# nalinbhardwaj/curdleproofs.pie

Measured on AMD Instinct MI355X. Metric: BLS12-381 G1 scalar-muls/sec at MSM size 2^20, higher is better.
Workload: dtype u32

## Files before the change

### curdleproofs_pie_amd/csrc/host_chains.h

```cpp
#pragma once

namespace cg1 {

static WinPlan make_plan(int c, bool glv = false) {
  WinPlan pl;
  const int bits = glv ? 127 : 255;
  pl.glv = glv ? 1 : 0;
  if (c > 0) { pl.cmax = c; pl.nwin = bits / c + 1; pl.n_hi = pl.nwin; }
  else {
    const int cm = -c, nw = (bits + 1 + cm - 1) / cm;
    pl.cmax = cm; pl.nwin = nw; pl.n_hi = bits + 1 - nw * (cm - 1);
    if (pl.n_hi < 0) pl.n_hi = 0;
  }
  return pl;
}

static int pick_plan_c(size_t n, int auto_plan) {
  const int c = pick_window(n);
  if (!auto_plan || c != 16) return c;
  if (n <= (1u << 14)) return -12;
  if (n <= (3u << 15)) return -13;
  if (n <= (3u << 16)) return -15;
  return 16;
}

int pick_window(size_t n) {
  if (n <= 128) return 4;
  if (n <= 8192) return 8;
  return 16;
}

static int wait_stream(Ctx* ctx) {
  if (ctx->blocking_sync) {
    HIPCHK(hipEventRecord(ctx->sync_ev, ctx->stream));
    HIPCHK(hipEventSynchronize(ctx->sync_ev));
    return CG1_OK;
  }
  HIPCHK(hipStreamSynchronize(ctx->stream));
  return CG1_OK;
}

struct PtSrc {
  enum Kind { AFFINE96 = 0, BLOBS = 1, PREPARED = 2 } kind = AFFINE96;
  const void* p = nullptr;
  const uint8_t* flags = nullptr;
  bool normalised = false;
  PtSrc() {}
  PtSrc(const void* affine96) : p(affine96) {}
};

static uint32_t blob_points_per_lane(size_t n) {
  size_t K = (n + (1u << 17) - 1) >> 17;
  return (uint32_t)(K < 1 ? 1 : (K > 16 ? 16 : K));
}

static void launch_prepare(hipStream_t st, const PtSrc& src, PreparedPoint* out, uint8_t* flags_out, uint32_t n32, uint32_t* status_words) {
  if (src.kind == PtSrc::AFFINE96) {
    hipLaunchKernelGGL(k_prepare_points, dim3((n32 + 255) / 256), dim3(256), 0, st, (const uint32_t*)src.p, out, flags_out, n32, status_words);
  } else if (src.normalised) {
    hipLaunchKernelGGL((k_prepare_blobs<false>), dim3((n32 + 127) / 128), dim3(128), 0, st, (const uint32_t*)src.p, out, flags_out, n32, 1u, status_words);
  } else {
    const uint32_t K = blob_points_per_lane(n32);
    const uint32_t lanes = (n32 + K - 1) / K;
    hipLaunchKernelGGL((k_prepare_blobs<true>), dim3((lanes + 127) / 128), dim3(128), 0, st, (const uint32_t*)src.p, out, flags_out, n32, K, status_words);
  }
}

struct ChainHooks {
  hipEvent_t before_start = nullptr, after_prepare = nullptr, before_accumulate = nullptr, after_accumulate = nullptr;
};

static int msm_enqueue(Ctx* ctx, const PtSrc& src, const void* d_scalars32, size_t n, const WinPlan& plan, int rank, int world,
                       const ChainHooks& hooks = ChainHooks()) {
  ctx->pend.active = false;
  HIPCHK(hipSetDevice(ctx->device));
  const int c = plan.cmax, nwin = plan.nwin;
  const size_t n_real = n;
  if (plan.glv) n *= 2;
  const int nlw = win_count(nwin, rank, world);
  if (nlw <= 0) return CG1_OK;
  const uint32_t NB = 1u << (c - 1);
  const uint32_t m = std::min<uint32_t>(ctx->seg_m, NB);
  const uint32_t J = NB / m;
  int nbits = 0; while ((1u << nbits) < J) ++nbits;
  const uint32_t bb = (uint32_t)c - 1u, lb2 = (bb + 1u) / 2u, hb2 = bb - lb2;
  const bool use2d = ctx->reduce_2d != 0;
  const uint32_t nitems = use2d ? 1u + hb2 + lb2 : 1u + (uint32_t)nbits;
  const size_t nb_total = (size_t)nlw * NB;
  uint32_t L0 = ctx->L0;
  while (L0 < 65536u && ((uint64_t)n * (uint64_t)nlw >> 18) > (uint64_t)L0) L0 <<= 1;
  if (ctx->chunk_rule && world == 1) {
    const uint64_t entries = (uint64_t)n * (uint64_t)nlw;
    if (entries >= (1ull << 20) && entries < (1ull << 21) && L0 < 10u) L0 = 10u;
    if (entries >= (1ull << 21) && entries < (1ull << 24) && nb_total > (size_t)ctx->rowcol_quad_max) {
      const double mload = (double)n / (double)(1u << bb);
      uint32_t want = (uint32_t)(mload + 8.0 * std::sqrt(mload) + 1.0);
      if (entries < (1ull << 22) && want > 20u) want = 20u;
      if (want > L0) L0 = want;
    }
  }
  int rc = ensure(ctx, n, nb_total, nlw, nitems, L0, src.kind != PtSrc::PREPARED);
  if (rc) return rc;
  hipStream_t st = ctx->stream;
  const uint32_t n32 = (uint32_t)n;
  const uint32_t gn = (n32 + 255) / 256;
  const int profile = ctx->profile;
  auto h0 = std::chrono::steady_clock::now();
  const bool resident = src.kind == PtSrc::PREPARED;
  const PreparedPoint* pts = resident ? static_cast<const PreparedPoint*>(src.p) : ctx->d_pts;
  const uint8_t* flags = resident ? src.flags : ctx->d_flags;
  const size_t nout_words = (size_t)nlw * nitems;
  uint32_t* bad_flag = reinterpret_cast<uint32_t*>(ctx->d_out + nout_words);
  if (hooks.before_start) HIPCHK(hipStreamWaitEvent(st, hooks.before_start, 0));
  if (profile >= 2) HIPCHK(hipEventRecord(ctx->ev[0], st));
  const uint32_t n_real32 = (uint32_t)n_real;
  if (resident) HIPCHK(hipMemsetAsync(bad_flag, 0, 16, st));
  else {
    launch_prepare(st, src, ctx->d_pts, ctx->d_flags, n_real32, bad_flag);
    if (plan.glv) hipLaunchKernelGGL(k_phi_records, dim3((n_real32 + 255) / 256), dim3(256), 0, st, ctx->d_pts, ctx->d_flags, n_real32);
  }
  if (hooks.after_prepare) HIPCHK(hipEventRecord(hooks.after_prepare, st));
  if (profile >= 2) HIPCHK(hipEventRecord(ctx->ev[1], st));
  const uint32_t nblk = (uint32_t)((nb_total + SCAN_ITEMS - 1) / SCAN_ITEMS);
  if (ctx->use_partition_sort && n <= PART_MAX_N) {
    const uint32_t want_sub = ctx->sort_sub_bits ? (uint32_t)ctx->sort_sub_bits : (n <= ((size_t)1 << 16) ? 7u : 8u);
    uint32_t sub_bits = bb < want_sub ? bb : want_sub;
    while (bb - sub_bits > 7u) ++sub_bits;
    const uint32_t nbins = 1u << (bb - sub_bits);
    const uint32_t nslices = (n32 + PART_TILE - 1) / PART_TILE;
    const uint32_t nbc = (uint32_t)nlw * nbins * nslices;
    hipLaunchKernelGGL(k_digits, dim3((n_real32 + 255) / 256), dim3(256), 0, st, (const uint32_t*)d_scalars32, flags, ctx->d_digits, n_real32, plan, rank, world, bad_flag);
    hipLaunchKernelGGL(k_part_count, dim3(nslices, nlw), dim3(256), 0, st, ctx->d_digits, ctx->d_blockcnt, n32, nslices, nbins, sub_bits);
    const uint32_t ublk = (nbc + SCAN_ITEMS - 1) / SCAN_ITEMS;
    if (ctx->scan_one && nbc <= USCAN1_MAX) {
      hipLaunchKernelGGL(k_uscan_one, dim3(1), dim3(1024), 0, st, ctx->d_blockcnt, nbc);
    } else {
      hipLaunchKernelGGL(k_uscan1, dim3(ublk), dim3(256), 0, st, ctx->d_blockcnt, ctx->d_ublocktot, nbc);
      hipLaunchKernelGGL(k_uscan2, dim3(1), dim3(256), 0, st, ctx->d_ublocktot, ublk, ctx->d_blockcnt, nbc);
      hipLaunchKernelGGL(k_uscan3, dim3(ublk), dim3(256), 0, st, ctx->d_ublocktot, ctx->d_blockcnt, nbc);
    }
    if (profile >= 2) HIPCHK(hipEventRecord(ctx->ev[2], st));
    hipLaunchKernelGGL(k_part_scatter, dim3(nslices, nlw), dim3(256), 0, st, ctx->d_digits, ctx->d_blockcnt, ctx->d_part, n32, nslices, nbins, sub_bits, ctx->stage_sort);
    const uint32_t nbt = (uint32_t)nlw * nbins;
    const int big_bins = ctx->big_bins && n32 > 2u * BIN_STAGE;
    hipLaunchKernelGGL(k_slice_plan, dim3(1), dim3(256), 0, st, ctx->d_blockcnt, nbt, nslices, ctx->d_slice_base, ctx->d_bigflag, big_bins);
    hipLaunchKernelGGL(k_bin_sort, dim3(nbt), dim3(256), 0, st, ctx->d_part, ctx->d_blockcnt, ctx->d_hist, ctx->d_sorted, nbt, nslices, sub_bits, ctx->stage_sort, ctx->d_bigflag);
    if (big_bins) {
      const uint32_t max_slices = (uint32_t)(((size_t)n * (size_t)nlw) / SLICE + nbt + 1);
      hipLaunchKernelGGL(k_slice_count, dim3(max_slices), dim3(256), 0, st, ctx->d_part, ctx->d_blockcnt, nbt, nslices, ctx->d_slice_base, ctx->d_slicehist);
      hipLaunchKernelGGL(k_slice_prefix, dim3(nbt), dim3(256), 0, st, ctx->d_blockcnt, nslices, sub_bits, ctx->d_slice_base, ctx->d_bigflag, ctx->d_slicehist, ctx->d_subbase, ctx->d_hist);
      hipLaunchKernelGGL(k_slice_scatter, dim3(max_slices), dim3(256), 0, st, ctx->d_part, ctx->d_blockcnt, nbt, nslices, ctx->d_slice_base, ctx->d_slicehist, ctx->d_subbase, ctx->d_sorted);
    }
    if (profile >= 2) HIPCHK(hipEventRecord(ctx->ev[3], st));
    if (ctx->scan_one && nb_total <= SCAN1_MAX) {
      hipLaunchKernelGGL(k_scan_one, dim3(1), dim3(1024), 0, st, ctx->d_hist, ctx->d_off, ctx->d_choff, (uint32_t)nb_total, L0);
    } else {
      hipLaunchKernelGGL(k_scan1, dim3(nblk), dim3(256), 0, st, ctx->d_hist, ctx->d_off, ctx->d_choff, ctx->d_blocktot, (uint32_t)nb_total, L0);
      hipLaunchKernelGGL(k_scan2, dim3(1), dim3(256), 0, st, ctx->d_blocktot, nblk, ctx->d_off, ctx->d_choff, (uint32_t)nb_total);
      hipLaunchKernelGGL(k_scan3, dim3(nblk), dim3(256), 0, st, ctx->d_blocktot, ctx->d_off, ctx->d_choff, (uint32_t)nb_total);
    }
  } else {
    HIPCHK(hipMemsetAsync(ctx->d_hist, 0, nb_total * 4, st));
    hipLaunchKernelGGL(k_hist, dim3(gn), dim3(256), 0, st, (const uint32_t*)d_scalars32, flags, ctx->d_hist, n32, plan, rank, world, bad_flag);
    if (profile >= 2) HIPCHK(hipEventRecord(ctx->ev[2], st));
    hipLaunchKernelGGL(k_scan1, dim3(nblk), dim3(256), 0, st, ctx->d_hist, ctx->d_off, ctx->d_choff, ctx->d_blocktot, (uint32_t)nb_total, L0);
    hipLaunchKernelGGL(k_scan2, dim3(1), dim3(256), 0, st, ctx->d_blocktot, nblk, ctx->d_off, ctx->d_choff, (uint32_t)nb_total);
    hipLaunchKernelGGL(k_scan3, dim3(nblk), dim3(256), 0, st, ctx->d_blocktot, ctx->d_off, ctx->d_choff, (uint32_t)nb_total);
    if (profile >= 2) HIPCHK(hipEventRecord(ctx->ev[3], st));
    hipLaunchKernelGGL(k_scatter, dim3(gn), dim3(256), 0, st, (const uint32_t*)d_scalars32, flags, ctx->d_hist, ctx->d_off, ctx->d_sorted, n32, plan, rank, world);
  }
  HIPCHK(hipMemsetAsync(ctx->d_zblock, 0, zblock_clear_bytes(ctx), st));
  hipLaunchKernelGGL(k_chunk_desc, dim3((uint32_t)std::min<size_t>(CHUNK_DESC_BLOCKS, (nb_total + 255) / 256)), dim3(256), 0, st, ctx->d_off, ctx->d_choff, ctx->d_desc, ctx->d_lenhist, ctx->d_heavy, (uint32_t)ctx->cap_heavy, (uint32_t)nb_total, L0, ctx->d_any_multi);
  const size_t max_chunks = nb_total + (n * (size_t)nlw) / L0 + 1;
  const uint32_t gchunks = (uint32_t)((max_chunks + 255) / 256);
  hipLaunchKernelGGL(k_len_scan, dim3(1), dim3(256), 0, st, ctx->d_lenhist, ctx->d_lenhist + LEN_BINS, ctx->d_off + nb_total, ctx->d_choff + nb_total, bad_flag);
  hipLaunchKernelGGL(k_order, dim3((gchunks + ORDER_PER - 1) / ORDER_PER), dim3(256), 0, st, ctx->d_desc, ctx->d_choff + nb_total, ctx->d_lenhist + LEN_BINS, ctx->d_order);
  if (hooks.before_accumulate) HIPCHK(hipStreamWaitEvent(st, hooks.before_accumulate, 0));
  if (profile >= 1) HIPCHK(hipEventRecord(ctx->ev[4], st));
  hipLaunchKernelGGL(k_accumulate, dim3(gchunks), dim3(256), 0, st, ctx->d_desc, ctx->d_choff + nb_total, ctx->d_order, ctx->d_sorted, pts, ctx->d_sums);
  if (profile >= 1) HIPCHK(hipEventRecord(ctx->ev[5], st));
  if (hooks.after_accumulate) HIPCHK(hipEventRecord(hooks.after_accumulate, st));
  hipLaunchKernelGGL(k_heavy_combine, dim3(512), dim3(256), 0, st, ctx->d_heavy, (uint32_t)ctx->cap_heavy, ctx->d_choff, ctx->d_sums, ctx->d_combined);
  const bool small_quad = ctx->quad && ctx->rowcol_quad && nb_total <= (size_t)ctx->rowcol_quad_max;
  const bool rows_fold = small_quad && use2d && ctx->rowcol_row && ctx->tree_row && nb_total <= 8192;
  if (rows_fold) {}
  else if (small_quad && ctx->fold_quad)
    hipLaunchKernelGGL(k_bucket_fold_quad, dim3((uint32_t)((nb_total * 4 + 255) / 256)), dim3(256), 0, st, ctx->d_choff, ctx->d_sums, ctx->d_combined, (uint32_t)nb_total, ctx->d_any_multi);
  else if (ctx->fold_pass)
    hipLaunchKernelGGL(k_bucket_fold, dim3((uint32_t)((nb_total + 255) / 256)), dim3(256), 0, st, ctx->d_choff, ctx->d_sums, ctx->d_combined, (uint32_t)nb_total, ctx->d_any_multi);
  bool tree_exports = false;
  if (use2d) {
    const uint32_t R = 1u << hb2, Cn = 1u << lb2;
    const uint32_t lpr = Cn < 32u ? Cn : 32u, lpc = R < 16u ? R : 16u;
    const uint32_t nrow_blocks = ((uint32_t)nlw * R + (256u / lpr) - 1u) / (256u / lpr);
    const uint32_t ncol_blocks = ((uint32_t)nlw * Cn + (256u / lpc) - 1u) / (256u / lpc);
    PointSum* rowsum = ctx->d_segrun;
    PointSum* colsum = ctx->d_segtot;
    if (small_quad) {
      uint32_t lgq = (R == Cn) ? 2u : 3u;
      if (ctx->rowcol_lgq >= 2 && ctx->rowcol_lgq <= 4) lgq = (uint32_t)ctx->rowcol_lgq;
      const uint32_t rc_waves = ((uint32_t)nlw * (R + Cn) + (16u >> lgq) - 1u) / (16u >> lgq);
      if (ctx->rowcol_row && ctx->tree_row)
        hipLaunchKernelGGL(k_rowcol_quad_row, dim3(((uint32_t)nlw * (R + Cn) + 3u) / 4u), dim3(256), 0, st, ctx->d_choff, ctx->d_sums, ctx->d_combined,
                           rowsum, colsum, (uint32_t)nlw, hb2, lb2);
      else
      hipLaunchKernelGGL(k_rowcol_quad, dim3((rc_waves + 3u) / 4u), dim3(256), 0, st, ctx->d_choff, ctx->d_sums,
                         rowsum, colsum, (uint32_t)nlw, hb2, lb2, lgq);
    }
    else
      hipLaunchKernelGGL(k_rowcol, dim3(nrow_blocks + ncol_blocks), dim3(256), 0, st, ctx->d_choff, ctx->d_sums, ctx->d_combined,
                         rowsum, colsum, (uint32_t)nlw, hb2, lb2, nrow_blocks, ctx->quad);
    if (profile >= 2) HIPCHK(hipEventRecord(ctx->ev[6], st));
    const uint32_t tree_threads = std::min<uint32_t>(512u, std::max<uint32_t>(64u, 4u << std::max(hb2, lb2)) >> (ctx->tree_shift >= 0 ? ctx->tree_shift : (ctx->tree_half ? 1 : 0)));
    if (ctx->tree_row) {
      uint32_t W = (1u << std::max(hb2, lb2)) >> 3;
      W = W < 1u ? 1u : (W > 16u ? 16u : W);
      tree_exports = ctx->zero_copy != 0;
      if (tree_exports) ++ctx->seq;
      hipLaunchKernelGGL(k_small_tree_row, dim3(nitems, nlw), dim3(64u * W), 0, st, rowsum, colsum, ctx->d_out, hb2, lb2,
                         tree_exports ? ctx->h_out_dev : (PointWords*)nullptr, bad_flag, ctx->h_flag_dev, ctx->seq);
    }
    else if (ctx->quad) hipLaunchKernelGGL(k_small_tree_quad, dim3(nitems, nlw), dim3(std::max<uint32_t>(64u, tree_threads)), 0, st, rowsum, colsum, ctx->d_out, hb2, lb2);
    else hipLaunchKernelGGL(k_small_tree, dim3(nitems, nlw), dim3(256), 0, st, rowsum, colsum, ctx->d_out, hb2, lb2);
  } else {
    const uint32_t nseg_total = (uint32_t)(nb_total / m);
    hipLaunchKernelGGL(k_seg_reduce, dim3((nseg_total + 255) / 256), dim3(256), 0, st, ctx->d_choff, ctx->d_sums, ctx->d_combined, ctx->d_segrun, ctx->d_segtot, nseg_total, m);
    if (profile >= 2) HIPCHK(hipEventRecord(ctx->ev[6], st));
    uint32_t S = (J + BT_ELEMS - 1) / BT_ELEMS; if (S < 1) S = 1; if (S > 64) S = 64;
    hipLaunchKernelGGL(k_bit_tree, dim3(nitems, nlw, S), dim3(256), 0, st, ctx->d_segrun, ctx->d_segtot, ctx->d_partial, J);
    hipLaunchKernelGGL(k_bit_tree_final, dim3((uint32_t)(nitems * nlw)), dim3(64), 0, st, ctx->d_partial, ctx->d_out, S);
  }
  const bool zc = ctx->zero_copy != 0;
  if (zc && tree_exports) {
  } else if (zc) {
    ++ctx->seq;
    const uint32_t nvec = (uint32_t)((((size_t)nlw * nitems + 1) * sizeof(PointWords)) / 16);
    hipLaunchKernelGGL(k_export_host, dim3(1), dim3(1024), 0, st, reinterpret_cast<const uint4*>(ctx->d_out), reinterpret_cast<uint4*>(ctx->h_out_dev), nvec,
                       ctx->h_flag_dev, ctx->seq);
  } else {
    HIPCHK(hipMemcpyAsync(ctx->h_out, ctx->d_out, ((size_t)nlw * nitems + 1) * sizeof(PointWords), hipMemcpyDeviceToHost, st));
  }
  if (profile >= 2) HIPCHK(hipEventRecord(ctx->ev[7], st));
  auto h1 = std::chrono::steady_clock::now();
  Ctx::Pending& pd = ctx->pend;
  pd.zero_copy = zc; pd.seq = ctx->seq; pd.hout = ctx->h_out;
  pd.active = true; pd.c = c; pd.plan = plan; pd.rank = rank; pd.world = world; pd.nlw = nlw; pd.nbits = nbits; pd.m = m; pd.lb2 = lb2; pd.hb2 = hb2;
  pd.nitems = nitems; pd.use2d = use2d; pd.profile = profile; pd.nout_words = nout_words; pd.h0 = h0; pd.h1 = h1;
  pd.arm_helpers = ctx->arm_helpers && ctx->host_split && ctx->horner_threads > 1 && n <= ((size_t)1 << 18);
  return CG1_OK;
}

static int msm_finish(Ctx* ctx, cg1h::jac& result) {
  result = cg1h::jac_identity();
  if (!ctx->pend.active) return CG1_OK;
  const Ctx::Pending pd = ctx->pend;
  ctx->pend.active = false;
  const int c = pd.c, rank = pd.rank, world = pd.world, nlw = pd.nlw, nbits = pd.nbits;
  (void)c;
  const uint32_t m = pd.m, lb2 = pd.lb2, hb2 = pd.hb2, nitems = pd.nitems;
  const bool use2d = pd.use2d;
  const size_t nout_words = pd.nout_words;
  const auto h0 = pd.h0, h1 = pd.h1;
  HIPCHK(hipSetDevice(ctx->device));
  struct StandDown { Ctx* c; bool on; ~StandDown() { if (on) for (int j = 0; j < 3; ++j) c->helper[j].disarm(); } } stand_down{ctx, false};
  if (pd.zero_copy && !ctx->blocking_sync && pd.profile < 2) {
    if (pd.arm_helpers) for (int j = 0; j < 3 && j + 1 < ctx->horner_threads; ++j) ctx->helper[j].arm();
    stand_down.on = pd.arm_helpers;
    volatile uint32_t* flag = ctx->h_flag;
    for (uint32_t spins = 0; *flag != pd.seq; ++spins) {
      if ((spins & 0x3fffu) == 0x3fffu) {
        hipError_t q = hipStreamQuery(ctx->stream);
        if (q == hipSuccess) { if (*flag != pd.seq) { snprintf(ctx->err, sizeof ctx->err, "the stream drained without the export flag"); return CG1_ERR_HIP; } break; }
        if (q != hipErrorNotReady) { snprintf(ctx->err, sizeof ctx->err, "stream failed: %s", hipGetErrorString(q)); return CG1_ERR_HIP; }
      }
      __builtin_ia32_pause();
    }
    std::atomic_thread_fence(std::memory_order_acquire);
  } else {
    int wrc = wait_stream(ctx); if (wrc) return wrc;
  }
  HIPCHK(hipGetLastError());
  {
    const uint32_t* st_words = reinterpret_cast<const uint32_t*>(pd.hout + nout_words);
    ctx->last_entries = st_words[1]; ctx->last_chunks = st_words[2];
    if (st_words[0]) {
      snprintf(ctx->err, sizeof ctx->err, "a scalar is >= 2^255: scalar32 must be a canonical Fr element (< r)");
      return CG1_ERR_ENCODING;
    }
  }
  auto h2 = std::chrono::steady_clock::now();
  { int erc = read_phase_events(ctx, pd.profile); if (erc) return erc; }
  ctx->last_c = c;

  auto t0 = std::chrono::steady_clock::now();
  ctx->host_ms[0] = std::chrono::duration<float, std::milli>(h1 - h0).count();
  ctx->host_ms[1] = std::chrono::duration<float, std::milli>(h2 - h1).count();
  ctx->host_ms[2] = std::chrono::duration<float, std::milli>(t0 - h2).count();
  int lm = 0; while ((1u << lm) < m) ++lm;
  const WinPlan& plan = pd.plan;
  constexpr int EMAX = 2 * 256 + 64;
  std::vector<std::pair<int, const PointWords*>> items;
  items.reserve((size_t)nlw * nitems);
  int e_top = 0;
  for (int lw = 0; lw < nlw; ++lw) {
    const int w = win_global(lw, rank, world), base = plan.off(w);
    const PointWords* row = pd.hout + (size_t)lw * nitems;
    auto put = [&](int e, const PointWords* p) { if (!p->inf && e >= 0 && e < EMAX) { items.emplace_back(e, p); if (e > e_top) e_top = e; } };
    put(base, &row[0]);
    if (use2d) {
      for (uint32_t k = 0; k < hb2; ++k) put(base + (int)lb2 + (int)k, &row[1 + k]);
      for (uint32_t k = 0; k < lb2; ++k) put(base + (int)k, &row[1 + hb2 + k]);
    } else {
      for (int b2 = 0; b2 < nbits; ++b2) put(base + lm + b2, &row[1 + b2]);
    }
  }
  uint16_t first[EMAX + 1];
  memset(first, 0, sizeof first);
  for (const auto& it : items) ++first[it.first + 1];
  for (int e = 0; e < EMAX; ++e) first[e + 1] = (uint16_t)(first[e + 1] + first[e]);
  std::vector<const PointWords*> byexp(items.size());
  {
    uint16_t cur[EMAX];
    memcpy(cur, first, sizeof cur);
    for (const auto& it : items) byexp[cur[it.first]++] = it.second;
  }
  auto horner = [&](int lo, int hi) {
    cg1h::jac a = cg1h::jac_identity();
    for (int e = hi; e >= lo; --e) {
      a = cg1h::jac_dbl(a);
      for (uint16_t k = first[e]; k < first[e + 1]; ++k) a = cg1h::jac_add(a, jac_from_words(*byexp[k]));
    }
    return a;
  };
  cg1h::jac acc;
  const int nth = (!ctx->host_split || e_top < 96) ? 1 : (ctx->horner_threads >= 4 && e_top >= 112 ? 4 : 2);
  if (nth > 1) {
    cg1h::jac part[4];
    int lo[5];
    {
      constexpr long DBL = 7, ADD = 16;
      auto fill = [&](long C, int* cut) {
        int e = 0;
        for (int j = 0; j < nth; ++j) {
          cut[j] = e;
          long adds = 0;
          while (e <= e_top && DBL * (e + 1) + ADD * (adds + (first[e + 1] - first[e])) <= C) { adds += first[e + 1] - first[e]; ++e; }
        }
        cut[nth] = e_top + 1;
        return e > e_top;
      };
      long lo_c = DBL * (e_top + 1), hi_c = DBL * (e_top + 1) + ADD * (long)items.size();
      int cut[5];
      while (lo_c < hi_c) {
        const long mid = (lo_c + hi_c) / 2;
        if (fill(mid, cut)) hi_c = mid; else lo_c = mid + 1;
      }
      fill(hi_c, cut);
      for (int j = 0; j <= nth; ++j) lo[j] = cut[j];
    }
    auto run_part = [&](int j) {
      cg1h::jac a = horner(lo[j], lo[j + 1] - 1);
      for (int k = 0; k < lo[j]; ++k) a = cg1h::jac_dbl(a);
      part[j] = a;
    };
    for (int j = 0; j + 1 < nth; ++j) ctx->helper[j].run([&, j]() { run_part(j); });
    if (pd.arm_helpers) for (int j = nth - 1 < 0 ? 0 : nth - 1; j < 3; ++j) ctx->helper[j].disarm();
    run_part(nth - 1);
    acc = part[nth - 1];
    for (int j = 0; j + 1 < nth; ++j) { ctx->helper[j].wait(); acc = cg1h::jac_add(acc, part[j]); }
  } else {
    if (pd.arm_helpers) for (int j = 0; j < 3; ++j) ctx->helper[j].disarm();
    acc = horner(0, e_top);
  }
  result = acc;
  ctx->host_tail_ms = std::chrono::duration<float, std::milli>(std::chrono::steady_clock::now() - t0).count();
  ctx->host_ms[3] = ctx->host_tail_ms;
  return CG1_OK;
}

static int pick_small_c(size_t n) {
  if (n <= 24) return 4;
  if (n <= 96) return 6;
  if (n <= 6 * SM_SLICE) return 7;
  return 8;
}

static int msm_enqueue_small(Ctx* ctx, const PtSrc& src, const void* d_scalars32, size_t n, int c, uint32_t M = 1, const uint32_t* d_offs = nullptr, size_t max_n = 0,
                             bool glv = false) {
  ctx->pend.active = false;
  HIPCHK(hipSetDevice(ctx->device));
  const WinPlan plan = make_plan(c, glv);
  const uint32_t nwin = (uint32_t)plan.nwin, bb = (uint32_t)c - 1u, lb2 = (bb + 1u) / 2u, hb2 = bb - lb2, nitems = 1u + hb2 + lb2;
  if (M == 1) max_n = n;
  const uint32_t S = (uint32_t)(((glv ? 2 * max_n : max_n) + SM_SLICE - 1) / SM_SLICE);
  auto h0 = std::chrono::steady_clock::now();
  if (!ctx->h_small_out) {
    HIPCHK(hipHostMalloc((void**)&ctx->h_small_out, ((size_t)SM_MAX_MSMS * 64 * 9 + 1) * sizeof(PointWords), hipHostMallocMapped | hipHostMallocCoherent));
    HIPCHK(hipHostGetDevicePointer((void**)&ctx->h_small_out_dev, ctx->h_small_out, 0));
    HIPCHK(hipMalloc(&ctx->d_small_ctr, (SM_MAX_MSMS * 64 + 8) * 4));
    HIPCHK(hipMemsetAsync(ctx->d_small_ctr, 0, (SM_MAX_MSMS * 64 + 8) * 4, ctx->stream));
  }
  const size_t need_partial = (size_t)M * nwin * S * nitems;
  if (S > 1 && need_partial > ctx->cap_small_partial) {
    if (ctx->d_small_partial) (void)hipFree(ctx->d_small_partial);
    ctx->d_small_partial = nullptr; ctx->cap_small_partial = 0;
    HIPCHK(hipMalloc(&ctx->d_small_partial, need_partial * sizeof(PointSum)));
    ctx->cap_small_partial = need_partial;
  }
  hipStream_t st = ctx->stream;
  SmallArgs a;
  a.src = src.p; a.flags = src.flags; a.scalars = static_cast<const uint32_t*>(d_scalars32); a.offs = d_offs;
  a.n = (uint32_t)n; a.M = M; a.S = S; a.c = (uint32_t)c; a.nwin = nwin; a.hb = hb2; a.lb = lb2; a.nitems = nitems;
  a.partial = ctx->d_small_partial; a.counters = ctx->d_small_ctr;
  a.out_host = ctx->h_small_out_dev; a.flag_host = ctx->h_flag_dev; a.seq = ++ctx->seq;
  a.row_tail = ctx->small_row_tail ? 1u : 0u;
  a.glv = glv ? 1u : 0u;
  int kind = (int)src.kind;
  if (src.kind == PtSrc::BLOBS && !src.normalised) {
    if (n > ctx->cap_small_pts) {
      if (ctx->d_small_pts) (void)hipFree(ctx->d_small_pts);
      if (ctx->d_small_flags) (void)hipFree(ctx->d_small_flags);
      ctx->d_small_pts = nullptr; ctx->d_small_flags = nullptr; ctx->cap_small_pts = 0;
      const size_t cap = n < SM_MAX_N ? SM_MAX_N : n;
      HIPCHK(hipMalloc(&ctx->d_small_pts, cap * sizeof(PreparedPoint)));
      HIPCHK(hipMalloc(&ctx->d_small_flags, cap + 16));
      ctx->cap_small_pts = cap;
    }
    launch_prepare(st, src, ctx->d_small_pts, ctx->d_small_flags, (uint32_t)n, nullptr);
    a.src = ctx->d_small_pts; a.flags = ctx->d_small_flags;
    kind = (int)PtSrc::PREPARED;
  }
  const dim3 grid(nwin, S, M), block(512);
  if (kind == (int)PtSrc::AFFINE96) hipLaunchKernelGGL((k_msm_small<0>), grid, block, 0, st, a);
  else if (kind == (int)PtSrc::BLOBS) hipLaunchKernelGGL((k_msm_small<1>), grid, block, 0, st, a);
  else hipLaunchKernelGGL((k_msm_small<2>), grid, block, 0, st, a);
  auto h1 = std::chrono::steady_clock::now();
  Ctx::Pending& pd = ctx->pend;
  pd.zero_copy = true; pd.seq = ctx->seq; pd.hout = ctx->h_small_out;
  pd.active = true; pd.c = c; pd.plan = plan; pd.rank = 0; pd.world = 1; pd.nlw = (int)nwin; pd.nbits = 0; pd.m = 1; pd.lb2 = lb2; pd.hb2 = hb2;
  pd.nitems = nitems; pd.use2d = true; pd.profile = 0; pd.nout_words = (size_t)M * nwin * nitems; pd.h0 = h0; pd.h1 = h1;
  pd.arm_helpers = ctx->arm_helpers && ctx->host_split && ctx->horner_threads > 1 && M == 1;
  return CG1_OK;
}

static cg1h::jac horner_2d_items(const PointWords* rows, const WinPlan& plan, uint32_t nitems, uint32_t hb2, uint32_t lb2) {
  constexpr int EMAX = 2 * 256 + 64;
  std::vector<std::pair<int, const PointWords*>> items;
  items.reserve((size_t)plan.nwin * nitems);
  int e_top = 0;
  for (int w = 0; w < plan.nwin; ++w) {
    const int base = plan.off(w);
    const PointWords* row = rows + (size_t)w * nitems;
    auto put = [&](int e, const PointWords* p) { if (!p->inf) { items.emplace_back(e, p); if (e > e_top) e_top = e; } };
    put(base, &row[0]);
    for (uint32_t k = 0; k < hb2; ++k) put(base + (int)lb2 + (int)k, &row[1 + k]);
    for (uint32_t k = 0; k < lb2; ++k) put(base + (int)k, &row[1 + hb2 + k]);
  }
  uint16_t first[EMAX + 1];
  memset(first, 0, sizeof first);
  for (const auto& it : items) ++first[it.first + 1];
  for (int e = 0; e < EMAX; ++e) first[e + 1] = (uint16_t)(first[e + 1] + first[e]);
  std::vector<const PointWords*> byexp(items.size());
  {
    uint16_t cur[EMAX];
    memcpy(cur, first, sizeof cur);
    for (const auto& it : items) byexp[cur[it.first]++] = it.second;
  }
  cg1h::jac a = cg1h::jac_identity();
  for (int e = e_top; e >= 0; --e) {
    a = cg1h::jac_dbl(a);
    for (uint16_t k = first[e]; k < first[e + 1]; ++k) a = cg1h::jac_add(a, jac_from_words(*byexp[k]));
  }
  return a;
}

static int msm_small_batched_finish(Ctx* ctx, uint32_t M, std::vector<cg1h::jac>& results) {
  const Ctx::Pending pd = ctx->pend;
  ctx->pend.active = false;
  HIPCHK(hipSetDevice(ctx->device));
  if (!ctx->blocking_sync) {
    volatile uint32_t* flag = ctx->h_flag;
    for (uint32_t spins = 0; *flag != pd.seq; ++spins) {
      if ((spins & 0x3fffu) == 0x3fffu) {
        hipError_t q = hipStreamQuery(ctx->stream);
        if (q == hipSuccess) { if (*flag != pd.seq) { snprintf(ctx->err, sizeof ctx->err, "the stream drained without the export flag"); return CG1_ERR_HIP; } break; }
        if (q != hipErrorNotReady) { snprintf(ctx->err, sizeof ctx->err, "stream failed: %s", hipGetErrorString(q)); return CG1_ERR_HIP; }
      }
      __builtin_ia32_pause();
    }
    std::atomic_thread_fence(std::memory_order_acquire);
  } else {
    int wrc = wait_stream(ctx); if (wrc) return wrc;
  }
  HIPCHK(hipGetLastError());
  const uint32_t* st_words = reinterpret_cast<const uint32_t*>(pd.hout + pd.nout_words);
  ctx->last_entries = st_words[1]; ctx->last_chunks = 0;
  if (st_words[0]) {
    snprintf(ctx->err, sizeof ctx->err, "a scalar is >= 2^255: scalar32 must be a canonical Fr element (< r)");
    return CG1_ERR_ENCODING;
  }
  auto t0 = std::chrono::steady_clock::now();
  const size_t per = (size_t)pd.plan.nwin * pd.nitems;
  auto one = [&](size_t j) { results[j] = horner_2d_items(pd.hout + j * per, pd.plan, pd.nitems, pd.hb2, pd.lb2); };
  if (M <= 4) {
    const size_t nth = std::min<size_t>(4, M);
    for (size_t t = 1; t < nth; ++t) ctx->helper[t - 1].run([&, t]() { for (size_t j = t; j < M; j += nth) one(j); });
    for (size_t j = 0; j < M; j += nth) one(j);
    for (size_t t = 1; t < nth; ++t) ctx->helper[t - 1].wait();
  } else {
    std::atomic<size_t> next{0};
    std::function<void()> work = [&]() { for (;;) { const size_t j = next.fetch_add(1); if (j >= M) return; one(j); } };
    Pool& pool = Pool::get();
    pool.run(work, std::min<size_t>(M, pool.size() + 1));
  }
  auto t1 = std::chrono::steady_clock::now();
  ctx->host_ms[0] = std::chrono::duration<float, std::milli>(pd.h1 - pd.h0).count();
  ctx->host_ms[1] = std::chrono::duration<float, std::milli>(t0 - pd.h1).count();
  ctx->host_ms[2] = 0;
  ctx->host_ms[3] = ctx->host_tail_ms = std::chrono::duration<float, std::milli>(t1 - t0).count();
  for (int i = 0; i < CG1_NPHASE; ++i) ctx->phase_ms[i] = 0.f;
  ctx->last_c = pd.c;
  ctx->last_acc_launches = 0;
  return CG1_OK;
}

static Ctx* child_of(Ctx* ctx);
static int msm_begin_split(Ctx* ctx, const PtSrc& src, const void* d_scalars32, size_t n, const WinPlan& plan, int rank, int world);

int msm_begin(Ctx* ctx, const PtSrc& src, const void* d_scalars32, size_t n, int c, int rank, int world) {
  ctx->pend.active = false;
  ctx->pend_c = 0;
  if (n == 0) return CG1_OK;
  if (n >= (1ull << 31)) { snprintf(ctx->err, sizeof ctx->err, "n too large"); return CG1_ERR_ARG; }
  if (world < 1 || world > 255 || rank < 0 || rank >= world) { snprintf(ctx->err, sizeof ctx->err, "bad window shard %d/%d", rank, world); return CG1_ERR_ARG; }
  for (int pass = (ctx->glv && 2 * n <= SM_MAX_N) ? 1 : 0; pass >= 0; --pass) {
    const bool sglv = pass == 1;
    const size_t nn = sglv ? 2 * n : n;
    const int bits = sglv ? 127 : 255;
    if (ctx->small_msm && nn <= SM_MAX_N && world == 1 && (c == 0 || (c >= 4 && c <= 9 && c != 5)) &&
        (size_t)(bits / (c ? c : pick_small_c(nn)) + 1) * ((nn + SM_SLICE - 1) / SM_SLICE) <= SM_ONE_ROUND) {
      if (c == 0) c = pick_small_c(nn);
      ctx->pend_c = c;
      return msm_enqueue_small(ctx, src, d_scalars32, n, c, 1, nullptr, 0, sglv);
    }
  }
  const bool glv = src.kind != PtSrc::PREPARED && ctx->use_partition_sort && 2 * n <= PART_MAX_N &&
                   (ctx->glv == 2 || (ctx->glv == 1 && n <= (size_t)ctx->glv_max_n));
  if (c == 0) c = pick_plan_c(glv ? 2 * n : n, ctx->auto_plan);
  const int cabs = c < 0 ? -c : c;
  if (cabs < 4 || cabs > 16) { snprintf(ctx->err, sizeof ctx->err, "window width %d out of range [4,16]", c); return CG1_ERR_ARG; }
  const WinPlan plan = make_plan(c, glv);
  ctx->pend_c = c;
  ctx->pend_split = false;
  if (ctx->split && n >= ctx->split_min_n && win_count(plan.nwin, rank, world) >= 2) return msm_begin_split(ctx, src, d_scalars32, n, plan, rank, world);
  return msm_enqueue(ctx, src, d_scalars32, n, plan, rank, world);
}
int msm_end(Ctx* ctx, cg1h::jac& result) {
  const bool was_small = ctx->pend.active && ctx->pend.hout == ctx->h_small_out;
  int rc = msm_finish(ctx, result);
  ctx->last_acc_launches = ctx->pend_split ? 2 : (was_small ? 0 : 1);
  if (ctx->pend_split) {
    ctx->pend_split = false;
    Ctx* ch = child_of(ctx);
    const float acc_hi = ctx->phase_ms[4], wait_hi = ctx->host_ms[1], tail_hi = ctx->host_ms[3], enq = ctx->host_ms[0];
    const uint32_t e_hi = ctx->last_entries, c_hi = ctx->last_chunks;
    cg1h::jac lo;
    int rc2 = msm_finish(ch, lo);
    if (rc == CG1_OK) rc = rc2;
    if (rc2 != CG1_OK) snprintf(ctx->err, sizeof ctx->err, "%s", ch->err);
    if (rc == CG1_OK) result = cg1h::jac_add(result, lo);
    for (int i = 0; i < CG1_NPHASE; ++i) ctx->phase_ms[i] += ch->phase_ms[i];
    ctx->phase_ms[4] = acc_hi + ch->phase_ms[4];
    ctx->last_entries = e_hi + ch->last_entries; ctx->last_chunks = c_hi + ch->last_chunks;
    ctx->host_ms[0] = enq + ch->host_ms[0]; ctx->host_ms[1] = wait_hi + ch->host_ms[1]; ctx->host_ms[3] = tail_hi + ch->host_ms[3];
    ctx->host_tail_ms = ch->host_ms[3];
  }
  if (ctx->pend_c) ctx->last_c = ctx->pend_c;
  return rc;
}
int msm_device(Ctx* ctx, const PtSrc& src, const void* d_scalars32, size_t n, int c, int rank, int world, cg1h::jac& result) {
  result = cg1h::jac_identity();
  int rc = msm_begin(ctx, src, d_scalars32, n, c, rank, world);
  if (rc) return rc;
  return msm_end(ctx, result);
}


int pick_window_batched(size_t n_avg, bool glv) {
  const int bits = glv ? 127 : 255;
  if (glv) n_avg *= 2;
  int best = 4; double best_cost = 1e300;
  for (int c = 4; c <= 9; ++c) {
    if (bits % c == 0) continue;
    int nwin = bits / c + 1;
    double NB = (double)(1u << (c - 1));
    double cost = (double)nwin * ((double)n_avg + 1.4 * (2.0 * NB + 3.0 * NB / 8.0)) + 1.4 * (double)bits;
    if (cost < best_cost) { best_cost = cost; best = c; }
  }
  return best;
}
int pick_window_batched(size_t n_avg) { return pick_window_batched(n_avg, false); }

static int ensure_child(Ctx* ctx);

struct BatchedChain {
  size_t M = 0; int c = 0; uint32_t nwin = 0; bool host_horner = false;
  std::chrono::steady_clock::time_point h0, h1;
};
static int batched_chain_enqueue(Ctx* ctx, const void* d_points96, const void* d_scalars32, const uint32_t* h_offsets, size_t M, int c, bool glv,
                                 hipEvent_t wait_before_accumulate, hipEvent_t record_after_accumulate, BatchedChain& bc) {
  const size_t N = h_offsets[M], N_real = N;
  HIPCHK(hipSetDevice(ctx->device));
  const WinPlan bplan = make_plan(c, glv);
  const uint32_t nwin = (uint32_t)bplan.nwin, NB = 1u << (c - 1);
  const size_t G = M * nwin, nb_total = G * NB;
  const size_t Nv = glv ? 2 * N : N;
  if (nb_total >= (1ull << 31) || Nv * nwin >= (1ull << 31)) { snprintf(ctx->err, sizeof ctx->err, "batch too large"); return CG1_ERR_ARG; }
  const uint32_t m = 8 < NB ? 8 : NB;
  uint32_t log2m = 0; while ((1u << log2m) < m) ++log2m;
  const uint32_t J = NB / m;
  uint32_t L0 = ctx->L0;
  while (L0 < 65536u && ((uint64_t)Nv * (uint64_t)nwin >> 18) > (uint64_t)L0) L0 <<= 1;
  int rc = ensure(ctx, Nv, nb_total, nwin, 1, L0);
  if (rc) return rc;
  if ((M + 1) > ctx->cap_boffs) {
    if (ctx->d_boffs) (void)hipFree(ctx->d_boffs);
    HIPCHK(hipMalloc(&ctx->d_boffs, (M + 1) * 4));
    ctx->cap_boffs = M + 1;
  }
  if (G > ctx->cap_gsum) {
    if (ctx->d_gsum) (void)hipFree(ctx->d_gsum);
    HIPCHK(hipMalloc(&ctx->d_gsum, G * sizeof(PointSum)));
    ctx->cap_gsum = G;
  }
  if (M > ctx->cap_bout) {
    if (ctx->d_bout) (void)hipFree(ctx->d_bout);
    if (ctx->h_bout) (void)hipHostFree(ctx->h_bout);
    HIPCHK(hipMalloc(&ctx->d_bout, (M + 1) * sizeof(PointWords)));
    HIPCHK(hipHostMalloc(&ctx->h_bout, (M + 1) * sizeof(PointWords)));
    ctx->cap_bout = M;
  }
  if (Nv * nwin > ctx->cap_digits) {
    if (ctx->d_digits) (void)hipFree(ctx->d_digits);
    HIPCHK(hipMalloc(&ctx->d_digits, Nv * nwin * 2 + 16));
    ctx->cap_digits = Nv * nwin;
  }
  hipStream_t st = ctx->stream;
  const uint32_t N32 = (uint32_t)N_real, gn = (N32 + 255) / 256, Nv32 = (uint32_t)Nv, split = glv ? N32 : 0u;
  auto h0 = std::chrono::steady_clock::now();
  HIPCHK(hipMemcpyAsync(ctx->d_boffs, h_offsets, (M + 1) * 4, hipMemcpyHostToDevice, st));
  if (ctx->profile >= 2) HIPCHK(hipEventRecord(ctx->ev[0], st));
  uint32_t* bad_flag = reinterpret_cast<uint32_t*>(ctx->d_bout + M);
  hipLaunchKernelGGL(k_prepare_points, dim3(gn), dim3(256), 0, st, (const uint32_t*)d_points96, ctx->d_pts, ctx->d_flags, N32, bad_flag);
  if (glv) hipLaunchKernelGGL(k_phi_records, dim3(gn), dim3(256), 0, st, ctx->d_pts, ctx->d_flags, N32);
  if (ctx->profile >= 2) HIPCHK(hipEventRecord(ctx->ev[1], st));
  hipLaunchKernelGGL(k_digits, dim3(gn), dim3(256), 0, st, (const uint32_t*)d_scalars32, ctx->d_flags, ctx->d_digits, N32, bplan, 0, 1, bad_flag);
  hipLaunchKernelGGL(k_group_count, dim3((uint32_t)M, nwin), dim3(256), 0, st, ctx->d_digits, ctx->d_boffs, ctx->d_hist, Nv32, NB, nwin, split);
  if (ctx->profile >= 2) HIPCHK(hipEventRecord(ctx->ev[2], st));
  const uint32_t nblk = (uint32_t)((nb_total + SCAN_ITEMS - 1) / SCAN_ITEMS);
  hipLaunchKernelGGL(k_scan1, dim3(nblk), dim3(256), 0, st, ctx->d_hist, ctx->d_off, ctx->d_choff, ctx->d_blocktot, (uint32_t)nb_total, L0);
  hipLaunchKernelGGL(k_scan2, dim3(1), dim3(256), 0, st, ctx->d_blocktot, nblk, ctx->d_off, ctx->d_choff, (uint32_t)nb_total);
  hipLaunchKernelGGL(k_scan3, dim3(nblk), dim3(256), 0, st, ctx->d_blocktot, ctx->d_off, ctx->d_choff, (uint32_t)nb_total);
  hipLaunchKernelGGL(k_group_scatter, dim3((uint32_t)M, nwin), dim3(256), 0, st, ctx->d_digits, ctx->d_boffs, ctx->d_off, ctx->d_sorted, Nv32, NB, nwin, split);
  if (ctx->profile >= 2) HIPCHK(hipEventRecord(ctx->ev[3], st));
  HIPCHK(hipMemsetAsync(ctx->d_zblock, 0, zblock_clear_bytes(ctx), st));
  hipLaunchKernelGGL(k_chunk_desc, dim3((uint32_t)std::min<size_t>(CHUNK_DESC_BLOCKS, (nb_total + 255) / 256)), dim3(256), 0, st, ctx->d_off, ctx->d_choff, ctx->d_desc, ctx->d_lenhist, ctx->d_heavy, (uint32_t)ctx->cap_heavy, (uint32_t)nb_total, L0, ctx->d_any_multi);
  const size_t max_chunks = nb_total + (Nv * (size_t)nwin) / L0 + 1;
  const uint32_t gchunks = (uint32_t)((max_chunks + 255) / 256);
  hipLaunchKernelGGL(k_len_scan, dim3(1), dim3(256), 0, st, ctx->d_lenhist, ctx->d_lenhist + LEN_BINS, ctx->d_off + nb_total, ctx->d_choff + nb_total, bad_flag);
  hipLaunchKernelGGL(k_order, dim3((gchunks + ORDER_PER - 1) / ORDER_PER), dim3(256), 0, st, ctx->d_desc, ctx->d_choff + nb_total, ctx->d_lenhist + LEN_BINS, ctx->d_order);
  if (wait_before_accumulate) HIPCHK(hipStreamWaitEvent(st, wait_before_accumulate, 0));
  if (ctx->profile >= 1) HIPCHK(hipEventRecord(ctx->ev[4], st));
  hipLaunchKernelGGL(k_accumulate, dim3(gchunks), dim3(256), 0, st, ctx->d_desc, ctx->d_choff + nb_total, ctx->d_order, ctx->d_sorted, ctx->d_pts, ctx->d_sums);
  if (ctx->profile >= 1) HIPCHK(hipEventRecord(ctx->ev[5], st));
  if (record_after_accumulate) HIPCHK(hipEventRecord(record_after_accumulate, st));
  const uint32_t nseg_total = (uint32_t)(nb_total / m);
  hipLaunchKernelGGL(k_heavy_combine, dim3(512), dim3(256), 0, st, ctx->d_heavy, (uint32_t)ctx->cap_heavy, ctx->d_choff, ctx->d_sums, ctx->d_combined);
  hipLaunchKernelGGL(k_seg_reduce, dim3((nseg_total + 255) / 256), dim3(256), 0, st, ctx->d_choff, ctx->d_sums, ctx->d_combined, ctx->d_segrun, ctx->d_segtot, nseg_total, m);
  hipLaunchKernelGGL(k_group_reduce, dim3((uint32_t)((G + 255) / 256)), dim3(256), 0, st, ctx->d_segrun, ctx->d_segtot, ctx->d_gsum, (uint32_t)G, J, log2m);
  if (ctx->profile >= 2) HIPCHK(hipEventRecord(ctx->ev[6], st));
  const bool host_horner = M <= (size_t)ctx->batched_host_horner_max;
  if (host_horner) {
    if (G > ctx->cap_gout) {
      if (ctx->d_gout) (void)hipFree(ctx->d_gout);
      if (ctx->h_gout) (void)hipHostFree(ctx->h_gout);
      ctx->d_gout = nullptr; ctx->h_gout = nullptr; ctx->cap_gout = 0;
      HIPCHK(hipMalloc(&ctx->d_gout, G * sizeof(PointWords)));
      HIPCHK(hipHostMalloc(&ctx->h_gout, G * sizeof(PointWords)));
      ctx->cap_gout = G;
    }
    hipLaunchKernelGGL(k_export_sums, dim3((uint32_t)((G + 63) / 64)), dim3(64), 0, st, ctx->d_gsum, ctx->d_gout, (uint32_t)G);
    HIPCHK(hipMemcpyAsync(ctx->h_gout, ctx->d_gout, G * sizeof(PointWords), hipMemcpyDeviceToHost, st));
    HIPCHK(hipMemcpyAsync(ctx->h_bout + M, ctx->d_bout + M, sizeof(PointWords), hipMemcpyDeviceToHost, st));
  } else {
    if (ctx->horner_row && M <= 2048) hipLaunchKernelGGL(k_msm_horner_row, dim3((uint32_t)M), dim3(64), 0, st, ctx->d_gsum, ctx->d_bout, (uint32_t)M, nwin, (uint32_t)c);
    else if (ctx->quad) hipLaunchKernelGGL(k_msm_horner_quad, dim3((uint32_t)((M * 4 + 63) / 64)), dim3(64), 0, st, ctx->d_gsum, ctx->d_bout, (uint32_t)M, nwin, (uint32_t)c);
    else hipLaunchKernelGGL(k_msm_horner, dim3((uint32_t)((M + 63) / 64)), dim3(64), 0, st, ctx->d_gsum, ctx->d_bout, (uint32_t)M, nwin, (uint32_t)c);
    HIPCHK(hipMemcpyAsync(ctx->h_bout, ctx->d_bout, (M + 1) * sizeof(PointWords), hipMemcpyDeviceToHost, st));
  }
  if (ctx->profile >= 2) HIPCHK(hipEventRecord(ctx->ev[7], st));
  bc.M = M; bc.c = c; bc.nwin = nwin; bc.host_horner = host_horner; bc.h0 = h0; bc.h1 = std::chrono::steady_clock::now();
  return CG1_OK;
}

static int batched_chain_finish(Ctx* ctx, const BatchedChain& bc, cg1h::jac* results) {
  const size_t M = bc.M; const int c = bc.c; const uint32_t nwin = bc.nwin; const bool host_horner = bc.host_horner;
  const auto h0 = bc.h0, h1 = bc.h1;
  HIPCHK(hipSetDevice(ctx->device));
  { int wrc = wait_stream(ctx); if (wrc) return wrc; }
  HIPCHK(hipGetLastError());
  {
    const uint32_t* st_words = reinterpret_cast<const uint32_t*>(ctx->h_bout + M);
    ctx->last_entries = st_words[1]; ctx->last_chunks = st_words[2];
    if (st_words[0]) {
      snprintf(ctx->err, sizeof ctx->err, "a scalar is >= 2^255: scalar32 must be a canonical Fr element (< r)");
      return CG1_ERR_ENCODING;
    }
  }
  auto h2 = std::chrono::steady_clock::now();
  { int erc = read_phase_events(ctx, ctx->profile); if (erc) return erc; }
  ctx->last_c = c;
  if (host_horner) {
    auto one = [&](size_t j) {
      cg1h::jac a = cg1h::jac_identity();
      for (int w = (int)nwin - 1; w >= 0; --w) {
        for (int k = 0; k < c; ++k) a = cg1h::jac_dbl(a);
        a = cg1h::jac_add(a, jac_from_words(ctx->h_gout[j * nwin + (size_t)w]));
      }
      results[j] = a;
    };
    const size_t nth = std::min<size_t>(4, M);
    for (size_t t = 1; t < nth; ++t) ctx->helper[t - 1].run([&, t]() { for (size_t j = t; j < M; j += nth) one(j); });
    for (size_t j = 0; j < M; j += nth) one(j);
    for (size_t t = 1; t < nth; ++t) ctx->helper[t - 1].wait();
  } else {
    for (size_t j = 0; j < M; ++j) results[j] = jac_from_words(ctx->h_bout[j]);
  }
  auto h3 = std::chrono::steady_clock::now();
  ctx->host_ms[0] = std::chrono::duration<float, std::milli>(h1 - h0).count();
  ctx->host_ms[1] = std::chrono::duration<float, std::milli>(h2 - h1).count();
  ctx->host_ms[2] = 0;
  ctx->host_ms[3] = ctx->host_tail_ms = std::chrono::duration<float, std::milli>(h3 - h2).count();
  return CG1_OK;
}

static int msm_batched_small_end(Ctx* ctx, size_t M, std::vector<cg1h::jac>& results) {
  if (M == 1) { cg1h::jac r; int rc = msm_finish(ctx, r); ctx->last_acc_launches = 0; if (rc == CG1_OK) results[0] = r; return rc; }
  return msm_small_batched_finish(ctx, (uint32_t)M, results);
}
int msm_batched_device(Ctx* ctx, const void* d_points96, const void* d_scalars32, const uint32_t* h_offsets, size_t M,
                       int c, std::vector<cg1h::jac>& results, bool* async_small = nullptr, const uint32_t* d_offsets_ready = nullptr) {
  if (async_small) *async_small = false;
  results.assign(M, cg1h::jac_identity());
  if (M == 0) return CG1_OK;
  const size_t N = h_offsets[M];
  for (size_t j = 0; j < M; ++j) if (h_offsets[j] > h_offsets[j + 1]) { snprintf(ctx->err, sizeof ctx->err, "offsets not monotone"); return CG1_ERR_ARG; }
  if (h_offsets[0] != 0) { snprintf(ctx->err, sizeof ctx->err, "offsets[0] must be 0"); return CG1_ERR_ARG; }
  if (N == 0) return CG1_OK;
  if (N >= (1ull << 31) || M > 65535) { snprintf(ctx->err, sizeof ctx->err, "batch too large"); return CG1_ERR_ARG; }
  {
    size_t max_n = 0;
    for (size_t j = 0; j < M; ++j) max_n = std::max<size_t>(max_n, h_offsets[j + 1] - h_offsets[j]);
    const bool sglv = ctx->glv && 2 * max_n <= SM_MAX_N;
    const size_t max_nn = sglv ? 2 * max_n : max_n;
    const int cs = c > 0 ? c : pick_small_c(max_nn);
    const size_t groups = (size_t)M * (size_t)((sglv ? 127 : 255) / cs + 1) * ((max_nn + SM_SLICE - 1) / SM_SLICE);
    if (ctx->small_msm && M <= SM_MAX_MSMS && max_nn <= SM_MAX_N && groups <= SM_MAX_GROUPS && cs >= 4 && cs <= 9 && cs != 5) {
      HIPCHK(hipSetDevice(ctx->device));
      const uint32_t* d_offs = d_offsets_ready;
      if (!d_offs) {
        if ((M + 1) > ctx->cap_boffs) {
          if (ctx->d_boffs) (void)hipFree(ctx->d_boffs);
          ctx->d_boffs = nullptr; ctx->cap_boffs = 0;
          HIPCHK(hipMalloc(&ctx->d_boffs, (M + 1) * 4));
          ctx->cap_boffs = M + 1;
        }
        HIPCHK(hipMemcpyAsync(ctx->d_boffs, h_offsets, (M + 1) * 4, hipMemcpyHostToDevice, ctx->stream));
        d_offs = ctx->d_boffs;
      }
      int rc = msm_enqueue_small(ctx, PtSrc(d_points96), d_scalars32, N, cs, (uint32_t)M, d_offs, max_n, sglv);
      if (rc) return rc;
      if (async_small) { *async_small = true; return CG1_OK; }
      return msm_batched_small_end(ctx, M, results);
    }
  }
  const bool glv = ctx->glv != 0 && 2 * N < (1ull << 31);
  if (c <= 0) c = pick_window_batched((N + M - 1) / M, glv);
  if (c < 4 || c > 9) { snprintf(ctx->err, sizeof ctx->err, "batched window width %d out of range [4,9]", c); return CG1_ERR_ARG; }
  HIPCHK(hipSetDevice(ctx->device));
  if (!ctx->batched_split || M < (size_t)ctx->batched_split_min_m || h_offsets[M / 2] == 0 || h_offsets[M / 2] == N) {
    BatchedChain bc;
    int rc = batched_chain_enqueue(ctx, d_points96, d_scalars32, h_offsets, M, c, glv, nullptr, nullptr, bc);
    if (rc) return rc;
    return batched_chain_finish(ctx, bc, results.data());
  }
  { int crc = ensure_child(ctx); if (crc) return crc; }
  Ctx* ch = child_of(ctx);
  ch->profile = ctx->profile; ch->L0 = ctx->L0; ch->quad = ctx->quad; ch->horner_row = ctx->horner_row; ch->blocking_sync = ctx->blocking_sync;
  ch->batched_host_horner_max = ctx->batched_host_horner_max; ch->use_partition_sort = ctx->use_partition_sort;
  const size_t Mlo = M / 2, Mhi = M - Mlo;
  std::vector<uint32_t> offs_hi(Mhi + 1);
  for (size_t j = 0; j <= Mhi; ++j) offs_hi[j] = h_offsets[Mlo + j] - h_offsets[Mlo];
  BatchedChain lo, hi;
  int rc = batched_chain_enqueue(ctx, d_points96, d_scalars32, h_offsets, Mlo, c, glv, nullptr, ctx->ev_acc, lo);
  if (rc) return rc;
  rc = batched_chain_enqueue(ch, static_cast<const uint8_t*>(d_points96) + 96ull * h_offsets[Mlo], static_cast<const uint8_t*>(d_scalars32) + 32ull * h_offsets[Mlo],
                             offs_hi.data(), Mhi, c, glv, ctx->ev_acc, nullptr, hi);
  if (rc) { snprintf(ctx->err, sizeof ctx->err, "%s", ch->err); (void)batched_chain_finish(ctx, lo, results.data()); return rc; }
  rc = batched_chain_finish(ctx, lo, results.data());
  const float acc_lo = ctx->phase_ms[4], enq_lo = ctx->host_ms[0], wait_lo = ctx->host_ms[1];
  const uint32_t e_lo = ctx->last_entries, c_lo = ctx->last_chunks;
  int rc2 = batched_chain_finish(ch, hi, results.data() + Mlo);
  if (rc2 != CG1_OK) snprintf(ctx->err, sizeof ctx->err, "%s", ch->err);
  if (rc == CG1_OK) rc = rc2;
  ctx->phase_ms[4] = acc_lo + ch->phase_ms[4];
  ctx->last_entries = e_lo + ch->last_entries; ctx->last_chunks = c_lo + ch->last_chunks;
  ctx->host_ms[0] = enq_lo + ch->host_ms[0]; ctx->host_ms[1] = wait_lo + ch->host_ms[1];
  return rc;
}

}
```

### curdleproofs_pie_amd/csrc/host_context.h

```cpp
#pragma once

namespace cg1 {

#define HIPCHK(x) do { hipError_t e_ = (x); if (e_ != hipSuccess) { \
  snprintf(ctx->err, sizeof ctx->err, "%s failed: %s (%s:%d)", #x, hipGetErrorString(e_), __FILE__, __LINE__); return CG1_ERR_HIP; } } while (0)

struct Helper {
  std::thread th;
  std::mutex mu;
  std::condition_variable cv;
  std::function<void()> job;
  bool has = false, done = true, quit = false, armed = false;
  std::atomic<bool> posted{false};
  std::atomic<bool> stand_down{false};
  void start_locked() { if (!th.joinable()) th = std::thread([this]() { loop(); }); }
  void run(std::function<void()> f) {
    std::unique_lock<std::mutex> lk(mu);
    start_locked();
    job = std::move(f); has = true; done = false;
    posted.store(true, std::memory_order_release);
    cv.notify_all();
  }
  void arm() {
    std::unique_lock<std::mutex> lk(mu);
    start_locked();
    if (!has && done) { stand_down.store(false, std::memory_order_relaxed); armed = true; cv.notify_all(); }
  }
  void disarm() { stand_down.store(true, std::memory_order_release); }
  void wait() {
    std::unique_lock<std::mutex> lk(mu);
    cv.wait(lk, [this]() { return done; });
  }
  void loop() {
    std::unique_lock<std::mutex> lk(mu);
    for (;;) {
      cv.wait(lk, [this]() { return has || quit || armed; });
      if (quit) return;
      if (!has) {
        armed = false;
        lk.unlock();
        const auto until = std::chrono::steady_clock::now() + std::chrono::milliseconds(2);
        for (uint32_t k = 0; !posted.load(std::memory_order_acquire); ++k) {
          if (stand_down.load(std::memory_order_acquire)) break;
          if ((k & 0xffu) == 0xffu && std::chrono::steady_clock::now() > until) break;
          __builtin_ia32_pause();
        }
        lk.lock();
        if (!has) continue;
      }
      armed = false;
      std::function<void()> f = std::move(job);
      has = false;
      posted.store(false, std::memory_order_relaxed);
      lk.unlock();
      f();
      lk.lock();
      done = true;
      cv.notify_all();
    }
  }
  ~Helper() {
    { std::unique_lock<std::mutex> lk(mu); quit = true; cv.notify_all(); }
    if (th.joinable()) th.join();
  }
};

struct Ctx {
  int device = 0;
  Helper helper[3];
  hipStream_t stream = nullptr;
  std::atomic<hipStream_t> copy_stream{nullptr};
  std::once_flag copy_once;
  hipEvent_t copy_ev = nullptr;
  std::vector<uint32_t> cu_mask;
  hipStream_t side_stream = nullptr;
  hipEvent_t side_ev = nullptr;
  hipEvent_t sync_ev = nullptr;
  int blocking_sync = 0;
  char err[256] = {0};
  size_t cap_n = 0, cap_nb = 0, cap_chunks = 0, cap_entries = 0, cap_out = 0;
  PreparedPoint* d_pts = nullptr;
  uint8_t* d_flags = nullptr;
  uint32_t *d_hist = nullptr, *d_off = nullptr, *d_choff = nullptr, *d_sorted = nullptr;
  uint2 *d_blocktot = nullptr, *d_desc = nullptr;
  uint32_t *d_order = nullptr, *d_lenhist = nullptr;
  uint32_t* d_zblock = nullptr; size_t cap_zblock = 0;
  uint32_t* d_any_multi = nullptr;
  PointSum* d_partial = nullptr; size_t cap_partial = 0;
  uint16_t* d_digits = nullptr; uint32_t* d_part = nullptr; uint32_t* d_blockcnt = nullptr; uint32_t* d_ublocktot = nullptr;
  size_t cap_digits = 0, cap_part = 0, cap_blockcnt = 0;
  uint32_t *d_slice_base = nullptr, *d_slicehist = nullptr, *d_subbase = nullptr; uint8_t* d_bigflag = nullptr;
  size_t cap_bigflag = 0, cap_slices = 0;
  int big_bins = 1;
  int use_partition_sort = 1;
  int stage_sort = 1;
  int host_split = 1;
  int rowcol_quad = 1;
  int rowcol_lgq = 0;
  int rowcol_quad_max = 1 << 18;
  int tree_shift = 2;
  int tree_half = 1;
  int merlin_sync = 1;
  uint32_t merlin_clk[2] = {0, 0};
  int fe_timed = 0;
  int fe_rows = 1;
  int fe_prio = 0;
  int decompress_waves = 3;
  void* d_opening = nullptr; size_t cap_opening = 0;
  void* d_prover = nullptr; size_t cap_prover = 0;
  PreparedPoint* d_gen_tab = nullptr;
  int fixed_slice = 0;
  int fixed_waves = 0;
  int ipa_inv = 0;
  int merlin_last_kernel = 0;
  int merlin_rows = 1;
  void* d_merlin_rows = nullptr; size_t merlin_rows_cap = 0;
  int merlin_lanes = 64;
  uint32_t merlin_passes = 0;
  int sort_sub_bits = 0;
  int batch_mul_host_max = -1;
  int last_batch_mul_on_host = 0;
  int batch_mul_quad_max = 8192;
  int scan_one = 1;
  int fold_pass = 1;
  int auto_plan = 1;
  struct Pending {
    bool active = false;
    int c = 0, rank = 0, world = 1, nlw = 0, nbits = 0;
    WinPlan plan;
    uint32_t m = 1, lb2 = 0, hb2 = 0, nitems = 0;
    bool use2d = true;
    int profile = 0;
    bool zero_copy = false; uint32_t seq = 0;
    bool arm_helpers = false;
    size_t nout_words = 0;
    const PointWords* hout = nullptr;
    std::chrono::steady_clock::time_point h0, h1;
  } pend;
  int split = 0;
  size_t split_min_n = (size_t)1 << 17;
  cg1_ctx* child = nullptr;
  hipEvent_t ev_prep = nullptr, ev_acc = nullptr;
  bool pend_split = false;
  int last_acc_launches = 0;
  int small_row_tail = 1;
  int small_msm = 1;
  PointSum* d_small_partial = nullptr; size_t cap_small_partial = 0;
  uint32_t* d_small_ctr = nullptr;
  PreparedPoint* d_small_pts = nullptr; uint8_t* d_small_flags = nullptr; size_t cap_small_pts = 0;
  PointWords* h_small_out = nullptr; PointWords* h_small_out_dev = nullptr;
  int quad = 1;
  int reduce_2d = 1;
  uint32_t* d_heavy = nullptr; size_t cap_heavy = 0;
  uint8_t* d_combined = nullptr; size_t cap_combined = 0;
  uint32_t* d_boffs = nullptr; size_t cap_boffs = 0;
  PointSum* d_gsum = nullptr; size_t cap_gsum = 0;
  PointWords* d_bout = nullptr; PointWords* h_bout = nullptr; size_t cap_bout = 0;
  PointWords* d_gout = nullptr; PointWords* h_gout = nullptr; size_t cap_gout = 0;
  int glv = 0;
  int glv_max_n = 1 << 14;
  int lincomb_zero_copy = 1;
  int fold_quad = 1;
  int rowcol_row = 1;
  int tree_row = 1;
  int horner_row = 1;
  int batch_mul_row = 1;
  int batched_split = 0;
  int batched_split_min_m = 256;
  int batched_host_horner_max = 24;
  PointSum *d_sums = nullptr, *d_segrun = nullptr, *d_segtot = nullptr;
  PointWords* d_out = nullptr;
  PointWords* h_out = nullptr;
  PointWords* h_out_dev = nullptr;
  uint32_t* h_flag = nullptr;
  uint32_t* h_flag_dev = nullptr;
  uint32_t seq = 0;
  int zero_copy = 1;
  int arm_helpers = 1;
  int horner_threads = 4;
  void* d_stage_pts = nullptr; void* d_stage_sc = nullptr; size_t cap_stage_pts = 0, cap_stage_sc = 0;
  uint8_t* h_lin = nullptr; uint8_t* h_lin_dev = nullptr; size_t cap_h_lin = 0;
  hipEvent_t ev[CG1_NPHASE + 1];
  float phase_ms[CG1_NPHASE] = {0};
  float host_tail_ms = 0;
  float host_ms[4] = {0, 0, 0, 0};
  int profile = 1;
  uint32_t last_chunks = 0, last_entries = 0;
  hipEvent_t tm_ev[2] = {nullptr, nullptr};
  int last_c = 0, pend_c = 0;
  int chunk_rule = 1;
  uint32_t L0 = 8;
  uint32_t seg_m = 4;
};

static void free_bufs(Ctx* c) {
  auto F = [](auto*& p) { if (p) { (void)hipFree(p); p = nullptr; } };
  F(c->d_pts); F(c->d_flags); F(c->d_hist); F(c->d_off); F(c->d_choff); F(c->d_sorted); F(c->d_blocktot); F(c->d_desc);
  F(c->d_sums); F(c->d_segrun); F(c->d_segtot); F(c->d_out); F(c->d_order); F(c->d_zblock); F(c->d_partial);
  c->d_lenhist = c->d_heavy = c->d_any_multi = nullptr; c->d_combined = nullptr; c->cap_zblock = 0; c->cap_heavy = 0; c->cap_combined = 0;
  c->cap_partial = 0;
  F(c->d_digits); F(c->d_part); F(c->d_blockcnt); F(c->d_ublocktot); F(c->d_boffs); F(c->d_gsum); F(c->d_bout);
  F(c->d_slice_base); F(c->d_slicehist); F(c->d_subbase); F(c->d_bigflag); c->cap_bigflag = 0; c->cap_slices = 0;
  if (c->h_bout) { (void)hipHostFree(c->h_bout); c->h_bout = nullptr; }
  if (c->h_lin) { (void)hipHostFree(c->h_lin); c->h_lin = nullptr; c->h_lin_dev = nullptr; c->cap_h_lin = 0; }
  if (c->d_gout) { (void)hipFree(c->d_gout); c->d_gout = nullptr; }
  if (c->h_gout) { (void)hipHostFree(c->h_gout); c->h_gout = nullptr; }
  c->cap_gout = 0;
  c->cap_boffs = c->cap_gsum = c->cap_bout = 0;
  c->cap_digits = c->cap_part = c->cap_blockcnt = 0;
  if (c->h_out) { (void)hipHostFree(c->h_out); c->h_out = nullptr; }
  c->cap_n = c->cap_nb = c->cap_chunks = c->cap_entries = c->cap_out = 0;
}

static int ensure(Ctx* ctx, size_t n, size_t nb_total, size_t nlw, size_t nitems, uint32_t L, bool need_points = true) {
  size_t entries = n * nlw;
  size_t chunks = nb_total + entries / L + 1;
  if (need_points && n > ctx->cap_n) {
    if (ctx->d_pts) (void)hipFree(ctx->d_pts);
    if (ctx->d_flags) (void)hipFree(ctx->d_flags);
    HIPCHK(hipMalloc(&ctx->d_pts, n * sizeof(PreparedPoint)));
    HIPCHK(hipMalloc(&ctx->d_flags, n + 16));
    ctx->cap_n = n;
  }
  if (nb_total > ctx->cap_nb) {
    auto F = [](auto*& p) { if (p) { (void)hipFree(p); p = nullptr; } };
    F(ctx->d_hist); F(ctx->d_off); F(ctx->d_choff); F(ctx->d_blocktot); F(ctx->d_segrun); F(ctx->d_segtot);
    HIPCHK(hipMalloc(&ctx->d_hist, nb_total * 4));
    HIPCHK(hipMalloc(&ctx->d_off, (nb_total + 1) * 4));
    HIPCHK(hipMalloc(&ctx->d_choff, (nb_total + 1) * 4));
    HIPCHK(hipMalloc(&ctx->d_blocktot, (nb_total / SCAN_ITEMS + 2) * sizeof(uint2)));
    HIPCHK(hipMalloc(&ctx->d_segrun, nb_total * sizeof(PointSum)));
    HIPCHK(hipMalloc(&ctx->d_segtot, nb_total * sizeof(PointSum)));
    ctx->cap_nb = nb_total;
  }
  if (entries > ctx->cap_entries) {
    if (ctx->d_sorted) (void)hipFree(ctx->d_sorted);
    HIPCHK(hipMalloc(&ctx->d_sorted, (entries + 1) * 4));
    ctx->cap_entries = entries;
  }
  if (chunks > ctx->cap_chunks) {
    if (ctx->d_desc) (void)hipFree(ctx->d_desc);
    if (ctx->d_sums) (void)hipFree(ctx->d_sums);
    if (ctx->d_order) (void)hipFree(ctx->d_order);
    HIPCHK(hipMalloc(&ctx->d_order, chunks * 4));
    HIPCHK(hipMalloc(&ctx->d_desc, chunks * sizeof(uint2)));
    HIPCHK(hipMalloc(&ctx->d_sums, chunks * sizeof(PointSum)));
    ctx->cap_chunks = chunks;
  }
  {
    const size_t hcap = entries / ((size_t)L * (HEAVY_MIN_CHUNKS - 1)) + 2;
    const size_t z0 = 2 * LEN_BINS + 1, h0 = z0 + (nb_total + 3) / 4, words = h0 + 1 + hcap + 64;
    if (words > ctx->cap_zblock) {
      if (ctx->d_zblock) (void)hipFree(ctx->d_zblock);
      ctx->d_zblock = nullptr; ctx->cap_zblock = 0;
      HIPCHK(hipMalloc(&ctx->d_zblock, words * 4));
      ctx->cap_zblock = words;
    }
    ctx->d_lenhist = ctx->d_zblock;
    ctx->d_any_multi = ctx->d_zblock + 2 * LEN_BINS;
    ctx->d_combined = reinterpret_cast<uint8_t*>(ctx->d_zblock + z0);
    ctx->d_heavy = ctx->d_zblock + h0;
    ctx->cap_heavy = hcap;
    ctx->cap_combined = nb_total;
  }
  if (ctx->use_partition_sort && n <= PART_MAX_N) {
    const size_t nslices = (n + PART_TILE - 1) / PART_TILE;
    const size_t nbc = nlw * 128 * nslices + 1;
    if (entries > ctx->cap_digits) {
      if (ctx->d_digits) (void)hipFree(ctx->d_digits);
      HIPCHK(hipMalloc(&ctx->d_digits, entries * 2 + 16));
      ctx->cap_digits = entries;
    }
    if (entries > ctx->cap_part) {
      if (ctx->d_part) (void)hipFree(ctx->d_part);
      HIPCHK(hipMalloc(&ctx->d_part, (entries + 1) * 4));
      ctx->cap_part = entries;
    }
    if (nlw * 128 > ctx->cap_bigflag) {
      auto F = [](auto*& p) { if (p) { (void)hipFree(p); p = nullptr; } };
      F(ctx->d_bigflag); F(ctx->d_slice_base); F(ctx->d_subbase);
      HIPCHK(hipMalloc(&ctx->d_bigflag, nlw * 128 + 16));
      HIPCHK(hipMalloc(&ctx->d_slice_base, (nlw * 128 + 1) * 4));
      HIPCHK(hipMalloc(&ctx->d_subbase, nlw * 128 * 256 * 4));
      ctx->cap_bigflag = nlw * 128;
    }
    {
      const size_t max_slices = entries / SLICE + nlw * 128 + 1;
      if (max_slices > ctx->cap_slices) {
        if (ctx->d_slicehist) (void)hipFree(ctx->d_slicehist);
        HIPCHK(hipMalloc(&ctx->d_slicehist, max_slices * 256 * 4));
        ctx->cap_slices = max_slices;
      }
    }
    if (nbc > ctx->cap_blockcnt) {
      if (ctx->d_blockcnt) (void)hipFree(ctx->d_blockcnt);
      if (ctx->d_ublocktot) (void)hipFree(ctx->d_ublocktot);
      HIPCHK(hipMalloc(&ctx->d_blockcnt, nbc * 4));
      HIPCHK(hipMalloc(&ctx->d_ublocktot, (nbc / SCAN_ITEMS + 2) * 4));
      ctx->cap_blockcnt = nbc;
    }
  }
  size_t nout = nlw * nitems;
  if (nout * 64 > ctx->cap_partial) {
    if (ctx->d_partial) (void)hipFree(ctx->d_partial);
    HIPCHK(hipMalloc(&ctx->d_partial, nout * 64 * sizeof(PointSum)));
    ctx->cap_partial = nout * 64;
  }
  if (nout > ctx->cap_out) {
    if (ctx->d_out) (void)hipFree(ctx->d_out);
    if (ctx->h_out) (void)hipHostFree(ctx->h_out);
    HIPCHK(hipMalloc(&ctx->d_out, (nout + 1) * sizeof(PointWords)));
    HIPCHK(hipHostMalloc(&ctx->h_out, (nout + 1) * sizeof(PointWords), hipHostMallocMapped | hipHostMallocCoherent));
    HIPCHK(hipHostGetDevicePointer((void**)&ctx->h_out_dev, ctx->h_out, 0));
    ctx->cap_out = nout;
  }
  return CG1_OK;
}

static size_t zblock_clear_bytes(const Ctx* ctx) {
  size_t bytes = (size_t)((ctx->d_heavy + 1) - ctx->d_zblock) * 4;
  bytes = (bytes + 255) & ~(size_t)255;
  const size_t cap = ctx->cap_zblock * 4;
  return bytes < cap ? bytes : cap;
}

static int read_phase_events(Ctx* ctx, int profile) {
  for (int i = 0; i < CG1_NPHASE; ++i) ctx->phase_ms[i] = 0.f;
  if (profile >= 2) {
    for (int i = 0; i < CG1_NPHASE; ++i) HIPCHK(hipEventElapsedTime(&ctx->phase_ms[i], ctx->ev[i], ctx->ev[i + 1]));
  } else if (profile == 1) {
    HIPCHK(hipEventElapsedTime(&ctx->phase_ms[4], ctx->ev[4], ctx->ev[5]));
  }
  return CG1_OK;
}

static cg1h::fe fe_from_words12(const uint32_t w[12]) {
  cg1h::fe r;
  for (int i = 0; i < 6; ++i) r.l[i] = (uint64_t)w[2 * i] | ((uint64_t)w[2 * i + 1] << 32);
  return r;
}
static cg1h::jac jac_from_words(const PointWords& p) {
  if (p.inf) return cg1h::jac_identity();
  return cg1h::jac_from_xyzz(fe_from_words12(p.w[0]), fe_from_words12(p.w[1]), fe_from_words12(p.w[2]), fe_from_words12(p.w[3]));
}

}
```

### curdleproofs_pie_amd/csrc/kernels_accumulate.h

```cpp
#pragma once

__global__ void __launch_bounds__(256) k_accumulate(const uint2* __restrict__ desc, const uint32_t* __restrict__ total_chunks,
                                                    const uint32_t* __restrict__ order, const uint32_t* __restrict__ sorted,
                                                    const PreparedPoint* __restrict__ pts, PointSum* __restrict__ sums) {
  uint32_t g = blockIdx.x * 256 + threadIdx.x;
  if (g >= *total_chunks) return;
  const uint32_t t = order[g];
  const uint2 d = desc[t];
  const uint32_t* ent = sorted + d.x;
  if (d.y == 0u) { store_sum(sums + t, xyzz_identity()); return; }
  uint32_t e = ent[0];
  fp x, y; uint32_t flags;
  load_affine(pts + (e & 0x7fffffffu), x, y, flags);
  xyzz acc;
  uint32_t j = 1;
  if (e >> 31) y = fp_neg<3>(y);
  if (d.y >= 2u) {
    const uint32_t e1 = ent[1];
    fp x1, y1;
    load_affine(pts + (e1 & 0x7fffffffu), x1, y1, flags);
    if (e1 >> 31) y1 = fp_neg<3>(y1);
    e = ent[d.y > 2u ? 2 : 1];
    fp xn, yn;
    load_affine(pts + (e & 0x7fffffffu), xn, yn, flags);
    acc = xyzz_mmadd(x, y, x1, y1);
    x = xn; y = yn;
    j = 2;
  } else {
    acc = xyzz_from_affine(x, y);
  }
  for (; j < d.y; ++j) {
    const uint32_t en = ent[(j + 1 < d.y) ? j + 1 : j];
    fp xn, yn;
    load_affine(pts + (en & 0x7fffffffu), xn, yn, flags);
    if (e >> 31) y = fp_neg<3>(y);
    if (!xyzz_madd_fast(acc, x, y)) break;
    e = en; x = xn; y = yn;
  }
  for (; j < d.y; ++j) {
    acc = xyzz_madd(acc, x, y);
    if (j + 1 < d.y) {
      e = ent[j + 1];
      load_affine(pts + (e & 0x7fffffffu), x, y, flags);
      if (e >> 31) y = fp_neg<3>(y);
    }
  }
  store_sum(sums + t, acc);
}

__global__ void __launch_bounds__(256) k_heavy_combine(const uint32_t* __restrict__ heavy, uint32_t heavy_cap,
                                                       const uint32_t* __restrict__ choff, PointSum* __restrict__ sums,
                                                       uint8_t* __restrict__ combined) {
  __shared__ PointSum sh[4];
  uint32_t nheavy = heavy[0];
  if (nheavy > heavy_cap) nheavy = heavy_cap;
  for (uint32_t h = blockIdx.x; h < nheavy; h += gridDim.x) {
    const uint32_t b = heavy[1 + h];
    const uint32_t c0 = choff[b], c1 = choff[b + 1];
    xyzz acc = xyzz_identity();
    for (uint32_t k = c0 + threadIdx.x; k < c1; k += 256) acc = xyzz_add(acc, load_sum(sums + k));
    __syncthreads();
    for (int delta = 32; delta >= 1; delta >>= 1) {
      xyzz o = shfl_down_xyzz(acc, delta);
      if ((threadIdx.x & 63) < (uint32_t)delta) acc = xyzz_add(acc, o);
    }
    if ((threadIdx.x & 63) == 0) store_sum(&sh[threadIdx.x >> 6], acc);
    __syncthreads();
    if (threadIdx.x == 0) {
      for (int k = 1; k < 4; ++k) acc = xyzz_add(acc, load_sum(&sh[k]));
      store_sum(sums + c0, acc);
      combined[b] = 1;
    }
    __syncthreads();
  }
}

__global__ void __launch_bounds__(256) k_bucket_fold(const uint32_t* __restrict__ choff, PointSum* __restrict__ sums,
                                                     uint8_t* __restrict__ combined, uint32_t nb_total, const uint32_t* __restrict__ any_multi = nullptr) {
  if (any_multi && *any_multi == 0u) return;
  uint32_t b = blockIdx.x * 256 + threadIdx.x;
  if (b >= nb_total) return;
  const uint32_t c0 = choff[b], c1 = choff[b + 1];
  if (c1 - c0 < 2u || c1 - c0 >= HEAVY_MIN_CHUNKS) return;
  xyzz acc = load_sum(sums + c0);
  for (uint32_t k = c0 + 1; k < c1; ++k) acc = xyzz_add(acc, load_sum(sums + k));
  store_sum(sums + c0, acc);
  combined[b] = 1;
}
```

### curdleproofs_pie_amd/csrc/kernels_sort.h

```cpp
#pragma once

constexpr uint32_t PART_TILE = 4096;
constexpr uint32_t PART_MAX_N = 1u << 23;

__device__ __forceinline__ uint32_t digit_mag(uint32_t e, uint32_t& neg) {
  if (e == 0x8000u) { neg = 0; return 0x8000u; }
  int d = (int)(int16_t)(uint16_t)e;
  neg = d < 0;
  return (uint32_t)(d < 0 ? -d : d);
}

__device__ int g_wave_agg = 1;
__device__ __forceinline__ uint32_t lds_ranked_inc(uint32_t* ctr, uint32_t key, bool active) {
  if (!g_wave_agg) return active ? atomicAdd(&ctr[key], 1u) : 0u;
  const unsigned long long amask = __ballot(active);
  if (amask == 0ull) return 0u;
  const int leader = __ffsll((long long)amask) - 1;
  const uint32_t k0 = __shfl(key, leader, 64);
  if (__ballot(active && key != k0) == 0ull) {
    const uint32_t lane = threadIdx.x & 63u;
    uint32_t base = 0;
    if ((int)lane == leader) base = atomicAdd(&ctr[k0], (uint32_t)__popcll(amask));
    base = __shfl(base, leader, 64);
    return base + (uint32_t)__popcll(amask & ((1ull << lane) - 1ull));
  }
  return active ? atomicAdd(&ctr[key], 1u) : 0u;
}

__global__ void __launch_bounds__(256) k_digits(const uint32_t* __restrict__ scalars, const uint8_t* __restrict__ inf_flag,
                                                uint16_t* __restrict__ digits, uint32_t n, WinPlan pl, int rank, int world,
                                                uint32_t* __restrict__ bad_flag) {
  uint32_t i = blockIdx.x * 256 + threadIdx.x;
  if (i >= n) return;
  const bool inf = inf_flag[i] != 0;
  DigitIter it;
  load_scalar(scalars, i, it);
  if (it.s[7] >> 31) *bad_flag = 1u;
  if (pl.glv) {
    GlvParts g;
    glv_split(it.s, g);
    DigitIter a, b;
    load_half(g.k1, g.neg1, a);
    load_half(g.k2, g.neg2, b);
    const size_t nv = 2 * (size_t)n;
    WinWalk ww(rank, world);
    for (int w = 0; w < pl.nwin; ++w) {
      const int d1 = a.next(pl, w), d2 = b.next(pl, w);
      const int lw = ww.step(w);
      if (lw < 0) continue;
      digits[(size_t)lw * nv + i] = inf ? (uint16_t)0 : (uint16_t)(d1 & 0xFFFF);
      digits[(size_t)lw * nv + n + i] = inf ? (uint16_t)0 : (uint16_t)(d2 & 0xFFFF);
    }
    return;
  }
  WinWalk ww(rank, world);
  for (int w = 0; w < pl.nwin; ++w) {
    int d = it.next(pl, w);
    const int lw = ww.step(w);
    if (lw < 0) continue;
    digits[(size_t)lw * n + i] = inf ? (uint16_t)0 : (uint16_t)(d & 0xFFFF);
  }
}

__global__ void __launch_bounds__(256) k_part_count(const uint16_t* __restrict__ digits, uint32_t* __restrict__ block_counts,
                                                    uint32_t n, uint32_t nslices, uint32_t nbins, uint32_t sub_bits) {
  __shared__ uint32_t cnt[128];
  if (threadIdx.x < 128) cnt[threadIdx.x] = 0;
  __syncthreads();
  const uint32_t slice = blockIdx.x, lw = blockIdx.y;
  const uint16_t* dg = digits + (size_t)lw * n;
  for (uint32_t k = 0; k < PART_TILE / 256; ++k) {
    uint32_t i = slice * PART_TILE + k * 256 + threadIdx.x;
    uint32_t e = (i < n) ? (uint32_t)dg[i] : 0u;
    uint32_t neg, key = e ? ((digit_mag(e, neg) - 1u) >> sub_bits) : 0u;
    lds_ranked_inc(cnt, key, e != 0u);
  }
  __syncthreads();
  if (threadIdx.x < nbins) block_counts[((size_t)lw * nbins + threadIdx.x) * nslices + slice] = cnt[threadIdx.x];
}

__global__ void __launch_bounds__(256) k_part_scatter(const uint16_t* __restrict__ digits, const uint32_t* __restrict__ block_base,
                                                      uint32_t* __restrict__ part, uint32_t n, uint32_t nslices, uint32_t nbins,
                                                      uint32_t sub_bits, int use_stage) {
  __shared__ uint32_t cur[128];
  __shared__ uint32_t gbase[128];
  __shared__ uint32_t lbase[128];
  __shared__ uint32_t stage[PART_TILE];
  __shared__ uint32_t gpos[PART_TILE];
  const uint32_t slice = blockIdx.x, lw = blockIdx.y;
  uint32_t mycnt = 0;
  if (threadIdx.x < nbins) {
    const size_t idx = ((size_t)lw * nbins + threadIdx.x) * nslices + slice;
    gbase[threadIdx.x] = block_base[idx];
    mycnt = block_base[idx + 1] - block_base[idx];
    lbase[threadIdx.x] = mycnt;
  } else if (threadIdx.x < 128) {
    lbase[threadIdx.x] = 0;
  }
  __syncthreads();
  if (use_stage) {
    for (int d = 1; d < 128; d <<= 1) {
      uint32_t u = (threadIdx.x < 128 && (int)threadIdx.x >= d) ? lbase[threadIdx.x - d] : 0u;
      __syncthreads();
      if (threadIdx.x < 128) lbase[threadIdx.x] += u;
      __syncthreads();
    }
    if (threadIdx.x < 128) { lbase[threadIdx.x] -= mycnt; cur[threadIdx.x] = lbase[threadIdx.x]; }
  } else if (threadIdx.x < nbins) {
    cur[threadIdx.x] = gbase[threadIdx.x];
  }
  __syncthreads();
  const uint16_t* dg = digits + (size_t)lw * n;
  const uint32_t sub_mask = (1u << sub_bits) - 1u;
  for (uint32_t k = 0; k < PART_TILE / 256; ++k) {
    uint32_t i = slice * PART_TILE + k * 256 + threadIdx.x;
    uint32_t e = (i < n) ? (uint32_t)dg[i] : 0u;
    uint32_t neg = 0, b = e ? (digit_mag(e, neg) - 1u) : 0u;
    const uint32_t bin = b >> sub_bits;
    uint32_t pos = lds_ranked_inc(cur, bin, e != 0u);
    const uint32_t val = i | (neg << 23) | ((b & sub_mask) << 24);
    if (e) {
      if (use_stage) { stage[pos] = val; gpos[pos] = gbase[bin] + (pos - lbase[bin]); }
      else part[pos] = val;
    }
  }
  if (use_stage) {
    __syncthreads();
    const uint32_t total = lbase[nbins - 1] + (block_base[((size_t)lw * nbins + nbins - 1) * nslices + slice + 1] - gbase[nbins - 1]);
    for (uint32_t o = threadIdx.x; o < total; o += 256) part[gpos[o]] = stage[o];
  }
}
constexpr uint32_t BIN_STAGE = 12288;
__global__ void __launch_bounds__(256) k_bin_sort(const uint32_t* __restrict__ part, const uint32_t* __restrict__ block_base,
                                                  uint32_t* __restrict__ hist, uint32_t* __restrict__ sorted,
                                                  uint32_t nbins_total, uint32_t nslices, uint32_t sub_bits, int use_stage,
                                                  const uint8_t* __restrict__ bigflag) {
  __shared__ uint32_t cnt[256];
  __shared__ uint32_t cur[256];
  __shared__ uint32_t stage[BIN_STAGE];
  const uint32_t g = blockIdx.x;
  if (bigflag[g]) return;
  const uint32_t start = block_base[(size_t)g * nslices];
  const uint32_t end = block_base[(size_t)(g + 1) * nslices];
  cnt[threadIdx.x] = 0;
  __syncthreads();
  const uint32_t span = ((end - start + 255u) / 256u) * 256u;
  for (uint32_t o = threadIdx.x; o < span; o += 256) {
    const bool live = start + o < end;
    lds_ranked_inc(cnt, live ? (part[start + o] >> 24) : 0u, live);
  }
  __syncthreads();
  const uint32_t mine = cnt[threadIdx.x];
  cur[threadIdx.x] = mine;
  __syncthreads();
  for (int d = 1; d < 256; d <<= 1) {
    uint32_t u = ((int)threadIdx.x >= d) ? cur[threadIdx.x - d] : 0u;
    __syncthreads();
    cur[threadIdx.x] += u;
    __syncthreads();
  }
  const uint32_t excl = cur[threadIdx.x] - mine;
  __syncthreads();
  const bool staged = use_stage && (end - start) <= BIN_STAGE;
  cur[threadIdx.x] = (staged ? 0u : start) + excl;
  if (threadIdx.x < (1u << sub_bits)) hist[((size_t)g << sub_bits) + threadIdx.x] = mine;
  __syncthreads();
  for (uint32_t o = threadIdx.x; o < span; o += 256) {
    const bool live = start + o < end;
    const uint32_t v = live ? part[start + o] : 0u;
    const uint32_t pos = lds_ranked_inc(cur, v >> 24, live);
    const uint32_t val = (v & 0x7fffffu) | ((v >> 23 & 1u) << 31);
    if (live) { if (staged) stage[pos] = val; else sorted[pos] = val; }
  }
  if (staged) {
    __syncthreads();
    for (uint32_t o = threadIdx.x; start + o < end; o += 256) sorted[start + o] = stage[o];
  }
}

constexpr uint32_t SLICE = BIN_STAGE;

__global__ void __launch_bounds__(256) k_slice_plan(const uint32_t* __restrict__ block_base, uint32_t nbins_total, uint32_t nslices,
                                                    uint32_t* __restrict__ slice_base ,
                                                    uint8_t* __restrict__ bigflag, int enable) {
  __shared__ uint32_t part_sum[256];
  const uint32_t per = (nbins_total + 255u) / 256u, g0 = threadIdx.x * per;
  uint32_t mine = 0;
  for (uint32_t g = g0; g < g0 + per && g < nbins_total; ++g) {
    const uint32_t size = block_base[(size_t)(g + 1) * nslices] - block_base[(size_t)g * nslices];
    mine += (enable && size > BIN_STAGE) ? (size + SLICE - 1u) / SLICE : 0u;
  }
  part_sum[threadIdx.x] = mine;
  __syncthreads();
  for (int d = 1; d < 256; d <<= 1) {
    uint32_t u = ((int)threadIdx.x >= d) ? part_sum[threadIdx.x - d] : 0u;
    __syncthreads();
    part_sum[threadIdx.x] += u;
    __syncthreads();
  }
  uint32_t run = part_sum[threadIdx.x] - mine;
  for (uint32_t g = g0; g < g0 + per && g < nbins_total; ++g) {
    const uint32_t size = block_base[(size_t)(g + 1) * nslices] - block_base[(size_t)g * nslices];
    const uint32_t ns = (enable && size > BIN_STAGE) ? (size + SLICE - 1u) / SLICE : 0u;
    slice_base[g] = run;
    bigflag[g] = ns ? 1 : 0;
    run += ns;
  }
  if (threadIdx.x == 255) slice_base[nbins_total] = part_sum[255];
}

__device__ __forceinline__ bool slice_of_block(const uint32_t* __restrict__ slice_base, uint32_t nbins_total, uint32_t b,
                                               uint32_t& g, uint32_t& s) {
  if (b >= slice_base[nbins_total]) return false;
  uint32_t lo = 0, hi = nbins_total;
  while (hi - lo > 1) {
    const uint32_t mid = (lo + hi) >> 1;
    if (slice_base[mid] <= b) lo = mid; else hi = mid;
  }
  g = lo;
  s = b - slice_base[lo];
  return true;
}

__global__ void __launch_bounds__(256) k_slice_count(const uint32_t* __restrict__ part, const uint32_t* __restrict__ block_base,
                                                     uint32_t nbins_total, uint32_t nslices, const uint32_t* __restrict__ slice_base,
                                                     uint32_t* __restrict__ slicehist) {
  __shared__ uint32_t cnt[256];
  uint32_t g, s;
  if (!slice_of_block(slice_base, nbins_total, blockIdx.x, g, s)) return;
  const uint32_t start = block_base[(size_t)g * nslices], end = block_base[(size_t)(g + 1) * nslices];
  const uint32_t lo = start + s * SLICE, hi = (lo + SLICE < end) ? lo + SLICE : end;
  cnt[threadIdx.x] = 0;
  __syncthreads();
  const uint32_t span = ((hi - lo + 255u) / 256u) * 256u;
  for (uint32_t o = threadIdx.x; o < span; o += 256) {
    const bool live = lo + o < hi;
    lds_ranked_inc(cnt, live ? (part[lo + o] >> 24) : 0u, live);
  }
  __syncthreads();
  slicehist[(size_t)blockIdx.x * 256u + threadIdx.x] = cnt[threadIdx.x];
}

__global__ void __launch_bounds__(256) k_slice_prefix(const uint32_t* __restrict__ block_base, uint32_t nslices, uint32_t sub_bits,
                                                      const uint32_t* __restrict__ slice_base, const uint8_t* __restrict__ bigflag,
                                                      uint32_t* __restrict__ slicehist, uint32_t* __restrict__ subbase,
                                                      uint32_t* __restrict__ hist) {
  __shared__ uint32_t tot[256];
  const uint32_t g = blockIdx.x;
  if (!bigflag[g]) return;
  const uint32_t b0 = slice_base[g], b1 = slice_base[g + 1];
  uint32_t run = 0;
  for (uint32_t b = b0; b < b1; ++b) {
    const size_t idx = (size_t)b * 256u + threadIdx.x;
    const uint32_t v = slicehist[idx];
    slicehist[idx] = run;
    run += v;
  }
  tot[threadIdx.x] = run;
  __syncthreads();
  for (int d = 1; d < 256; d <<= 1) {
    uint32_t u = ((int)threadIdx.x >= d) ? tot[threadIdx.x - d] : 0u;
    __syncthreads();
    tot[threadIdx.x] += u;
    __syncthreads();
  }
  subbase[(size_t)g * 256u + threadIdx.x] = block_base[(size_t)g * nslices] + tot[threadIdx.x] - run;
  if (threadIdx.x < (1u << sub_bits)) hist[((size_t)g << sub_bits) + threadIdx.x] = run;
}

__global__ void __launch_bounds__(256) k_slice_scatter(const uint32_t* __restrict__ part, const uint32_t* __restrict__ block_base,
                                                       uint32_t nbins_total, uint32_t nslices, const uint32_t* __restrict__ slice_base,
                                                       const uint32_t* __restrict__ slicehist, const uint32_t* __restrict__ subbase,
                                                       uint32_t* __restrict__ sorted) {
  __shared__ uint32_t cnt[256];
  __shared__ uint32_t cur[256];
  __shared__ uint32_t gdst[256];
  __shared__ uint32_t stage[SLICE];
  uint32_t g, s;
  if (!slice_of_block(slice_base, nbins_total, blockIdx.x, g, s)) return;
  const uint32_t start = block_base[(size_t)g * nslices], end = block_base[(size_t)(g + 1) * nslices];
  const uint32_t lo = start + s * SLICE, hi = (lo + SLICE < end) ? lo + SLICE : end;
  cnt[threadIdx.x] = 0;
  __syncthreads();
  const uint32_t span = ((hi - lo + 255u) / 256u) * 256u;
  for (uint32_t o = threadIdx.x; o < span; o += 256) {
    const bool live = lo + o < hi;
    lds_ranked_inc(cnt, live ? (part[lo + o] >> 24) : 0u, live);
  }
  __syncthreads();
  const uint32_t mine = cnt[threadIdx.x];
  __syncthreads();
  for (int d = 1; d < 256; d <<= 1) {
    uint32_t u = ((int)threadIdx.x >= d) ? cnt[threadIdx.x - d] : 0u;
    __syncthreads();
    cnt[threadIdx.x] += u;
    __syncthreads();
  }
  const uint32_t lbase = cnt[threadIdx.x] - mine;
  __syncthreads();
  cnt[threadIdx.x] = lbase;
  cur[threadIdx.x] = lbase;
  gdst[threadIdx.x] = subbase[(size_t)g * 256u + threadIdx.x] + slicehist[(size_t)blockIdx.x * 256u + threadIdx.x];
  __syncthreads();
  for (uint32_t o = threadIdx.x; o < span; o += 256) {
    const bool live = lo + o < hi;
    const uint32_t v = live ? part[lo + o] : 0u;
    const uint32_t pos = lds_ranked_inc(cur, v >> 24, live);
    if (live) stage[pos] = v;
  }
  __syncthreads();
  for (uint32_t o = threadIdx.x; o < hi - lo; o += 256) {
    const uint32_t v = stage[o], k = v >> 24;
    sorted[gdst[k] + (o - cnt[k])] = (v & 0x7fffffu) | ((v >> 23 & 1u) << 31);
  }
}

__global__ void __launch_bounds__(256) k_uscan1(uint32_t* __restrict__ a, uint32_t* __restrict__ block_tot, uint32_t n) {
  __shared__ uint32_t sh[256];
  uint32_t base = blockIdx.x * SCAN_ITEMS + threadIdx.x * 4;
  uint32_t v[4], local = 0;
#pragma unroll
  for (int k = 0; k < 4; ++k) { v[k] = (base + k < n) ? a[base + k] : 0u; local += v[k]; }
  sh[threadIdx.x] = local;
  __syncthreads();
  for (int d = 1; d < 256; d <<= 1) {
    uint32_t u = ((int)threadIdx.x >= d) ? sh[threadIdx.x - d] : 0u;
    __syncthreads();
    sh[threadIdx.x] += u;
    __syncthreads();
  }
  uint32_t excl = sh[threadIdx.x] - local;
#pragma unroll
  for (int k = 0; k < 4; ++k) { if (base + k < n) a[base + k] = excl; excl += v[k]; }
  if (threadIdx.x == 255) block_tot[blockIdx.x] = sh[255];
}
__global__ void __launch_bounds__(256) k_uscan2(uint32_t* __restrict__ block_tot, uint32_t nblocks, uint32_t* __restrict__ a, uint32_t n) {
  __shared__ uint32_t sh[256];
  uint32_t carry = 0;
  for (uint32_t tile = 0; tile < nblocks; tile += 256) {
    uint32_t i = tile + threadIdx.x;
    uint32_t v = (i < nblocks) ? block_tot[i] : 0u;
    sh[threadIdx.x] = v;
    __syncthreads();
    for (int d = 1; d < 256; d <<= 1) {
      uint32_t u = ((int)threadIdx.x >= d) ? sh[threadIdx.x - d] : 0u;
      __syncthreads();
      sh[threadIdx.x] += u;
      __syncthreads();
    }
    if (i < nblocks) block_tot[i] = carry + sh[threadIdx.x] - v;
    uint32_t tot = sh[255];
    __syncthreads();
    carry += tot;
  }
  if (threadIdx.x == 0) a[n] = carry;
}
__global__ void __launch_bounds__(256) k_uscan3(const uint32_t* __restrict__ block_tot, uint32_t* __restrict__ a, uint32_t n) {
  uint32_t base = blockIdx.x * SCAN_ITEMS + threadIdx.x * 4;
  uint32_t p = block_tot[blockIdx.x];
#pragma unroll
  for (int k = 0; k < 4; ++k) if (base + k < n) a[base + k] += p;
}

constexpr uint32_t USCAN1_MAX = 1u << 15;
__global__ void __launch_bounds__(1024) k_uscan_one(uint32_t* __restrict__ a, uint32_t n) {
  __shared__ uint32_t sh[1024];
  const uint32_t per = (n + 1023u) / 1024u, lo = threadIdx.x * per, hi = (lo + per < n) ? lo + per : n;
  uint32_t local = 0;
  for (uint32_t i = lo; i < hi; ++i) local += a[i];
  sh[threadIdx.x] = local;
  __syncthreads();
  for (int d = 1; d < 1024; d <<= 1) {
    uint32_t u = ((int)threadIdx.x >= d) ? sh[threadIdx.x - d] : 0u;
    __syncthreads();
    sh[threadIdx.x] += u;
    __syncthreads();
  }
  uint32_t excl = sh[threadIdx.x] - local;
  for (uint32_t i = lo; i < hi; ++i) { const uint32_t v = a[i]; a[i] = excl; excl += v; }
  if (threadIdx.x == 1023) a[n] = sh[1023];
}

__global__ void __launch_bounds__(256) k_group_count(const uint16_t* __restrict__ digits, const uint32_t* __restrict__ offs,
                                                     uint32_t* __restrict__ hist, uint32_t N, uint32_t NB, uint32_t nwin, uint32_t split) {
  __shared__ uint32_t cnt[256];
  cnt[threadIdx.x] = 0;
  __syncthreads();
  const uint32_t j = blockIdx.x, w = blockIdx.y;
  const uint32_t o0 = offs[j], o1 = offs[j + 1];
  const uint32_t span = ((o1 - o0 + 255u) / 256u) * 256u;
  for (uint32_t half = 0; half < (split ? 2u : 1u); ++half) {
    const uint16_t* dg = digits + (size_t)w * N + (size_t)half * split;
    for (uint32_t o = threadIdx.x; o < span; o += 256) {
      const uint32_t e = (o0 + o < o1) ? (uint32_t)dg[o0 + o] : 0u;
      uint32_t neg;
      lds_ranked_inc(cnt, e ? digit_mag(e, neg) - 1u : 0u, e != 0u);
    }
  }
  __syncthreads();
  if (threadIdx.x < NB) hist[((size_t)j * nwin + w) * NB + threadIdx.x] = cnt[threadIdx.x];
}

__global__ void __launch_bounds__(256) k_group_scatter(const uint16_t* __restrict__ digits, const uint32_t* __restrict__ offs,
                                                       const uint32_t* __restrict__ off, uint32_t* __restrict__ sorted,
                                                       uint32_t N, uint32_t NB, uint32_t nwin, uint32_t split) {
  __shared__ uint32_t cur[256];
  const uint32_t j = blockIdx.x, w = blockIdx.y;
  if (threadIdx.x < NB) cur[threadIdx.x] = off[((size_t)j * nwin + w) * NB + threadIdx.x];
  __syncthreads();
  const uint32_t o0 = offs[j], o1 = offs[j + 1];
  const uint16_t* dg = digits + (size_t)w * N;
  const uint32_t span = ((o1 - o0 + 255u) / 256u) * 256u;
  for (uint32_t half = 0; half < (split ? 2u : 1u); ++half) {
    for (uint32_t o = threadIdx.x; o < span; o += 256) {
      const uint32_t i = half * split + o0 + o;
      const uint32_t e = (o0 + o < o1) ? (uint32_t)dg[i] : 0u;
      uint32_t neg = 0;
      const uint32_t b = e ? digit_mag(e, neg) - 1u : 0u;
      const uint32_t pos = lds_ranked_inc(cur, b, e != 0u);
      if (e) sorted[pos] = i | (neg << 31);
    }
  }
}

__global__ void __launch_bounds__(256) k_group_reduce(const PointSum* __restrict__ seg_run, const PointSum* __restrict__ seg_tot,
                                                      PointSum* __restrict__ group_sum, uint32_t ngroups, uint32_t J, uint32_t log2m) {
  uint32_t g = blockIdx.x * 256 + threadIdx.x;
  if (g >= ngroups) return;
  const PointSum* run = seg_run + (size_t)g * J;
  const PointSum* tot = seg_tot + (size_t)g * J;
  xyzz r = xyzz_identity(), t = xyzz_identity();
  for (uint32_t s = J - 1; s >= 1; --s) { r = xyzz_add(r, load_sum(run + s)); t = xyzz_add(t, r); }
  for (uint32_t k = 0; k < log2m; ++k) t = xyzz_dbl(t);
  for (uint32_t s = 0; s < J; ++s) t = xyzz_add(t, load_sum(tot + s));
  store_sum(group_sum + g, t);
}

__global__ void __launch_bounds__(64) k_msm_horner(const PointSum* __restrict__ group_sum, PointWords* __restrict__ out,
                                                   uint32_t M, uint32_t nwin, uint32_t c) {
  uint32_t j = blockIdx.x * 64 + threadIdx.x;
  if (j >= M) return;
  xyzz acc = xyzz_identity();
  for (int w = (int)nwin - 1; w >= 0; --w) {
    for (uint32_t k = 0; k < c; ++k) acc = xyzz_dbl(acc);
    acc = xyzz_add(acc, load_sum(group_sum + (size_t)j * nwin + w));
  }
  xyzz_words o;
  xyzz_export(acc, o);
  PointWords* dst = out + j;
  for (int cidx = 0; cidx < 4; ++cidx) for (int k = 0; k < 12; ++k) dst->w[cidx][k] = o.w[cidx][k];
  dst->inf = o.inf;
}

constexpr uint32_t MAX_CHUNKS_PER_BUCKET = 4096;
constexpr uint32_t HEAVY_MIN_CHUNKS = 17;
__device__ __forceinline__ uint32_t chunk_len(uint32_t cnt, uint32_t L0) {
  uint32_t s = (cnt + MAX_CHUNKS_PER_BUCKET - 1) / MAX_CHUNKS_PER_BUCKET;
  return s > L0 ? s : L0;
}
__device__ __forceinline__ uint32_t chunk_count(uint32_t cnt, uint32_t L0) {
  if (cnt == 0) return 0;
  uint32_t L = chunk_len(cnt, L0);
  return (cnt + L - 1) / L;
}

__global__ void __launch_bounds__(256) k_scan1(const uint32_t* __restrict__ hist, uint32_t* __restrict__ off, uint32_t* __restrict__ choff,
                                               uint2* __restrict__ block_tot, uint32_t nb_total, uint32_t L0) {
  __shared__ uint2 sh[256];
  uint32_t base = blockIdx.x * SCAN_ITEMS + threadIdx.x * 4;
  uint32_t cnt[4], ch[4];
  uint2 local = make_uint2(0, 0);
#pragma unroll
  for (int k = 0; k < 4; ++k) {
    cnt[k] = (base + k < nb_total) ? hist[base + k] : 0u;
    ch[k] = chunk_count(cnt[k], L0);
    local.x += cnt[k]; local.y += ch[k];
  }
  sh[threadIdx.x] = local;
  __syncthreads();
  for (int d = 1; d < 256; d <<= 1) {
    uint2 v = make_uint2(0, 0);
    if ((int)threadIdx.x >= d) v = sh[threadIdx.x - d];
    __syncthreads();
    sh[threadIdx.x].x += v.x; sh[threadIdx.x].y += v.y;
    __syncthreads();
  }
  uint2 excl = make_uint2(sh[threadIdx.x].x - local.x, sh[threadIdx.x].y - local.y);
#pragma unroll
  for (int k = 0; k < 4; ++k) {
    if (base + k < nb_total) { off[base + k] = excl.x; choff[base + k] = excl.y; }
    excl.x += cnt[k]; excl.y += ch[k];
  }
  if (threadIdx.x == 255) block_tot[blockIdx.x] = sh[255];
}
__global__ void __launch_bounds__(256) k_scan2(uint2* __restrict__ block_tot, uint32_t nblocks, uint32_t* __restrict__ off,
                                               uint32_t* __restrict__ choff, uint32_t nb_total) {
  __shared__ uint2 sh[256];
  uint2 carry = make_uint2(0, 0);
  for (uint32_t tile = 0; tile < nblocks; tile += 256) {
    uint32_t i = tile + threadIdx.x;
    uint2 v = (i < nblocks) ? block_tot[i] : make_uint2(0, 0);
    sh[threadIdx.x] = v;
    __syncthreads();
    for (int d = 1; d < 256; d <<= 1) {
      uint2 u = make_uint2(0, 0);
      if ((int)threadIdx.x >= d) u = sh[threadIdx.x - d];
      __syncthreads();
      sh[threadIdx.x].x += u.x; sh[threadIdx.x].y += u.y;
      __syncthreads();
    }
    if (i < nblocks) block_tot[i] = make_uint2(carry.x + sh[threadIdx.x].x - v.x, carry.y + sh[threadIdx.x].y - v.y);
    uint2 tot = sh[255];
    __syncthreads();
    carry.x += tot.x; carry.y += tot.y;
  }
  if (threadIdx.x == 0) { off[nb_total] = carry.x; choff[nb_total] = carry.y; }
}
__global__ void __launch_bounds__(256) k_scan3(const uint2* __restrict__ block_tot, uint32_t* __restrict__ off,
                                               uint32_t* __restrict__ choff, uint32_t nb_total) {
  uint32_t base = blockIdx.x * SCAN_ITEMS + threadIdx.x * 4;
  uint2 p = block_tot[blockIdx.x];
#pragma unroll
  for (int k = 0; k < 4; ++k) if (base + k < nb_total) { off[base + k] += p.x; choff[base + k] += p.y; }
}

constexpr uint32_t LEN_BINS = 256;
__device__ __forceinline__ uint32_t len_key(uint32_t len) { return len < LEN_BINS - 1 ? len : LEN_BINS - 1; }

constexpr uint32_t SCAN1_MAX = 1u << 13;
__global__ void __launch_bounds__(1024) k_scan_one(const uint32_t* __restrict__ hist, uint32_t* __restrict__ off, uint32_t* __restrict__ choff,
                                                    uint32_t nb_total, uint32_t L0) {
  __shared__ uint2 sh[1024];
  const uint32_t per = (nb_total + 1023u) / 1024u, lo = threadIdx.x * per, hi = (lo + per < nb_total) ? lo + per : nb_total;
  uint2 local = make_uint2(0, 0);
  for (uint32_t i = lo; i < hi; ++i) { const uint32_t c = hist[i]; local.x += c; local.y += chunk_count(c, L0); }
  sh[threadIdx.x] = local;
  __syncthreads();
  for (int d = 1; d < 1024; d <<= 1) {
    uint2 v = make_uint2(0, 0);
    if ((int)threadIdx.x >= d) v = sh[threadIdx.x - d];
    __syncthreads();
    sh[threadIdx.x].x += v.x; sh[threadIdx.x].y += v.y;
    __syncthreads();
  }
  uint2 excl = make_uint2(sh[threadIdx.x].x - local.x, sh[threadIdx.x].y - local.y);
  for (uint32_t i = lo; i < hi; ++i) {
    const uint32_t c = hist[i];
    off[i] = excl.x; choff[i] = excl.y;
    excl.x += c; excl.y += chunk_count(c, L0);
  }
  if (threadIdx.x == 1023) { off[nb_total] = sh[1023].x; choff[nb_total] = sh[1023].y; }
}

constexpr uint32_t CHUNK_DESC_BLOCKS = 320;
__global__ void __launch_bounds__(256) k_chunk_desc(const uint32_t* __restrict__ off, const uint32_t* __restrict__ choff,
                                                    uint2* __restrict__ desc, uint32_t* __restrict__ len_hist,
                                                    uint32_t* __restrict__ heavy ,
                                                    uint32_t heavy_cap, uint32_t nb_total, uint32_t L0, uint32_t* __restrict__ any_multi = nullptr) {
  __shared__ uint32_t sh[LEN_BINS];
  sh[threadIdx.x] = 0;
  __syncthreads();
#pragma unroll 1
  for (uint32_t b = blockIdx.x * 256 + threadIdx.x; b - threadIdx.x < nb_total; b += gridDim.x * 256) {
  if (b < nb_total) {
    uint32_t start = off[b], cnt = off[b + 1] - start;
    if (cnt) {
      uint32_t L = chunk_len(cnt, L0), nch = (cnt + L - 1) / L, o = choff[b];
      for (uint32_t k = 0; k < nch; ++k) {
        uint32_t s = k * L, len = (cnt - s < L) ? (cnt - s) : L;
        desc[o + k] = make_uint2(start + s, len);
      }
      if (nch > 1u) atomicAdd(&sh[len_key(L)], nch - 1u);
      atomicAdd(&sh[len_key(cnt - (nch - 1u) * L)], 1u);
      if (nch >= HEAVY_MIN_CHUNKS) {
        uint32_t slot = atomicAdd(&heavy[0], 1u);
        if (slot < heavy_cap) heavy[1 + slot] = b;
      } else if (nch >= 2u && any_multi) {
        *any_multi = 1u;
      }
    }
  }
  }
  __syncthreads();
  uint32_t v = sh[threadIdx.x];
  if (v) atomicAdd(&len_hist[threadIdx.x], v);
}

__global__ void __launch_bounds__(256) k_len_scan(const uint32_t* __restrict__ len_hist, uint32_t* __restrict__ len_cursor,
                                                  const uint32_t* __restrict__ total_entries, const uint32_t* __restrict__ total_chunks,
                                                  uint32_t* __restrict__ stats) {
  __shared__ uint32_t sh[LEN_BINS];
  if (threadIdx.x == 0) { stats[1] = *total_entries; stats[2] = *total_chunks; }
  uint32_t rev = LEN_BINS - 1 - threadIdx.x;
  uint32_t v = len_hist[rev];
  sh[threadIdx.x] = v;
  __syncthreads();
  for (int d = 1; d < 256; d <<= 1) {
    uint32_t u = ((int)threadIdx.x >= d) ? sh[threadIdx.x - d] : 0u;
    __syncthreads();
    sh[threadIdx.x] += u;
    __syncthreads();
  }
  len_cursor[rev] = sh[threadIdx.x] - v;
}

constexpr uint32_t ORDER_PER = 8;
__global__ void __launch_bounds__(256) k_order(const uint2* __restrict__ desc, const uint32_t* __restrict__ total_chunks,
                                               uint32_t* __restrict__ len_cursor, uint32_t* __restrict__ order) {
  __shared__ uint32_t cnt[LEN_BINS];
  __shared__ uint32_t base[LEN_BINS];
  cnt[threadIdx.x] = 0;
  __syncthreads();
  const uint32_t total = *total_chunks;
  uint32_t key[ORDER_PER], local[ORDER_PER];
#pragma unroll
  for (uint32_t rep = 0; rep < ORDER_PER; ++rep) {
    const uint32_t t = (blockIdx.x * ORDER_PER + rep) * 256 + threadIdx.x;
    const bool live = t < total;
    key[rep] = live ? len_key(desc[t].y) : 0u;
    local[rep] = 0;
    const unsigned long long amask = __ballot(live);
    if (amask) {
      const int leader = __ffsll((long long)amask) - 1;
      const uint32_t k0 = __shfl(key[rep], leader, 64);
      const unsigned long long same = __ballot(live && key[rep] == k0);
      const uint32_t lane = threadIdx.x & 63u;
      uint32_t b0 = 0;
      if ((int)lane == leader) b0 = atomicAdd(&cnt[k0], (uint32_t)__popcll(same));
      b0 = __shfl(b0, leader, 64);
      if (live) local[rep] = (key[rep] == k0) ? b0 + (uint32_t)__popcll(same & ((1ull << lane) - 1ull)) : atomicAdd(&cnt[key[rep]], 1u);
    }
  }
  __syncthreads();
  const uint32_t c = cnt[threadIdx.x];
  if (c) base[threadIdx.x] = atomicAdd(&len_cursor[threadIdx.x], c);
  __syncthreads();
#pragma unroll
  for (uint32_t rep = 0; rep < ORDER_PER; ++rep) {
    const uint32_t t = (blockIdx.x * ORDER_PER + rep) * 256 + threadIdx.x;
    if (t < total) order[base[key[rep]] + local[rep]] = t;
  }
}
```

Before: 371.5 million.

## Fuse small pipeline kernels to cut launches in MSM sort/scan stages

Merges many small launches in the bucket-sort pipeline. Digit extraction is fused into partition counting for non-GLV plans. The second-level scans are folded into the third pass, with each block summing its predecessors' totals. The zblock memset moves into the scan kernels, the length scan moves into k_order, and heavy-combine is merged with bucket-fold into one k_chunk_join. The slice count and prefix steps are folded into part_scatter and bin_sort. The aim is to cut kernel-launch and serialization overhead, at the cost of redundant prefix reads per block and the length scan being recomputed in every k_order block.

```diff
diff --git a/curdleproofs_pie_amd/csrc/host_chains.h b/curdleproofs_pie_amd/csrc/host_chains.h
--- a/curdleproofs_pie_amd/csrc/host_chains.h
+++ b/curdleproofs_pie_amd/csrc/host_chains.h
@@ -122,6 +122,7 @@
   if (hooks.after_prepare) HIPCHK(hipEventRecord(hooks.after_prepare, st));
   if (profile >= 2) HIPCHK(hipEventRecord(ctx->ev[1], st));
   const uint32_t nblk = (uint32_t)((nb_total + SCAN_ITEMS - 1) / SCAN_ITEMS);
+  const uint32_t zwords = zblock_clear_words(ctx);
   if (ctx->use_partition_sort && n <= PART_MAX_N) {
     const uint32_t want_sub = ctx->sort_sub_bits ? (uint32_t)ctx->sort_sub_bits : (n <= ((size_t)1 << 16) ? 7u : 8u);
     uint32_t sub_bits = bb < want_sub ? bb : want_sub;
@@ -129,65 +130,65 @@
     const uint32_t nbins = 1u << (bb - sub_bits);
     const uint32_t nslices = (n32 + PART_TILE - 1) / PART_TILE;
     const uint32_t nbc = (uint32_t)nlw * nbins * nslices;
-    hipLaunchKernelGGL(k_digits, dim3((n_real32 + 255) / 256), dim3(256), 0, st, (const uint32_t*)d_scalars32, flags, ctx->d_digits, n_real32, plan, rank, world, bad_flag);
-    hipLaunchKernelGGL(k_part_count, dim3(nslices, nlw), dim3(256), 0, st, ctx->d_digits, ctx->d_blockcnt, n32, nslices, nbins, sub_bits);
+    if (plan.glv) {
+      hipLaunchKernelGGL(k_digits, dim3((n_real32 + 255) / 256), dim3(256), 0, st, (const uint32_t*)d_scalars32, flags, ctx->d_digits, n_real32, plan, rank, world, bad_flag);
+      hipLaunchKernelGGL(k_part_count, dim3(nslices, nlw), dim3(256), 0, st, ctx->d_digits, ctx->d_blockcnt, n32, nslices, nbins, sub_bits);
+    } else {
+      hipLaunchKernelGGL(k_part_count_scalars, dim3(nslices), dim3(PART_COUNT_THREADS), (size_t)nlw * nbins * 4, st, (const uint32_t*)d_scalars32, flags, ctx->d_digits,
+                         ctx->d_blockcnt, n32, nslices, nbins, sub_bits, (uint32_t)nlw, plan, rank, world, bad_flag);
+    }
     const uint32_t ublk = (nbc + SCAN_ITEMS - 1) / SCAN_ITEMS;
     if (ctx->scan_one && nbc <= USCAN1_MAX) {
       hipLaunchKernelGGL(k_uscan_one, dim3(1), dim3(1024), 0, st, ctx->d_blockcnt, nbc);
     } else {
       hipLaunchKernelGGL(k_uscan1, dim3(ublk), dim3(256), 0, st, ctx->d_blockcnt, ctx->d_ublocktot, nbc);
-      hipLaunchKernelGGL(k_uscan2, dim3(1), dim3(256), 0, st, ctx->d_ublocktot, ublk, ctx->d_blockcnt, nbc);
-      hipLaunchKernelGGL(k_uscan3, dim3(ublk), dim3(256), 0, st, ctx->d_ublocktot, ctx->d_blockcnt, nbc);
+      hipLaunchKernelGGL(k_uscan3, dim3(ublk), dim3(256), 0, st, ctx->d_ublocktot, ublk, ctx->d_blockcnt, nbc);
     }
     if (profile >= 2) HIPCHK(hipEventRecord(ctx->ev[2], st));
-    hipLaunchKernelGGL(k_part_scatter, dim3(nslices, nlw), dim3(256), 0, st, ctx->d_digits, ctx->d_blockcnt, ctx->d_part, n32, nslices, nbins, sub_bits, ctx->stage_sort);
     const uint32_t nbt = (uint32_t)nlw * nbins;
     const int big_bins = ctx->big_bins && n32 > 2u * BIN_STAGE;
-    hipLaunchKernelGGL(k_slice_plan, dim3(1), dim3(256), 0, st, ctx->d_blockcnt, nbt, nslices, ctx->d_slice_base, ctx->d_bigflag, big_bins);
-    hipLaunchKernelGGL(k_bin_sort, dim3(nbt), dim3(256), 0, st, ctx->d_part, ctx->d_blockcnt, ctx->d_hist, ctx->d_sorted, nbt, nslices, sub_bits, ctx->stage_sort, ctx->d_bigflag);
-    if (big_bins) {
-      const uint32_t max_slices = (uint32_t)(((size_t)n * (size_t)nlw) / SLICE + nbt + 1);
-      hipLaunchKernelGGL(k_slice_count, dim3(max_slices), dim3(256), 0, st, ctx->d_part, ctx->d_blockcnt, nbt, nslices, ctx->d_slice_base, ctx->d_slicehist);
-      hipLaunchKernelGGL(k_slice_prefix, dim3(nbt), dim3(256), 0, st, ctx->d_blockcnt, nslices, sub_bits, ctx->d_slice_base, ctx->d_bigflag, ctx->d_slicehist, ctx->d_subbase, ctx->d_hist);
-      hipLaunchKernelGGL(k_slice_scatter, dim3(max_slices), dim3(256), 0, st, ctx->d_part, ctx->d_blockcnt, nbt, nslices, ctx->d_slice_base, ctx->d_slicehist, ctx->d_subbase, ctx->d_sorted);
-    }
+    const uint32_t max_slices = big_bins ? (uint32_t)(((size_t)n * (size_t)nlw) / SLICE + nbt + 1) : 0u;
+    hipLaunchKernelGGL(k_part_scatter, dim3(nslices, nlw + (big_bins ? 1 : 0)), dim3(256), 0, st, ctx->d_digits, ctx->d_blockcnt, ctx->d_part, n32, nslices, nbins, sub_bits,
+                       ctx->stage_sort, nbt, ctx->d_slice_base);
+    hipLaunchKernelGGL(k_bin_sort, dim3(nbt + max_slices), dim3(256), 0, st, ctx->d_part, ctx->d_blockcnt, ctx->d_hist, ctx->d_sorted, nbt, nslices, sub_bits, ctx->stage_sort,
+                       big_bins, ctx->d_slice_base, ctx->d_slicehist);
+    if (big_bins)
+      hipLaunchKernelGGL(k_slice_scatter, dim3(max_slices), dim3(256), 0, st, ctx->d_part, ctx->d_blockcnt, nbt, nslices, sub_bits, ctx->d_slice_base, ctx->d_slicehist,
+                         ctx->d_hist, ctx->d_sorted);
     if (profile >= 2) HIPCHK(hipEventRecord(ctx->ev[3], st));
     if (ctx->scan_one && nb_total <= SCAN1_MAX) {
-      hipLaunchKernelGGL(k_scan_one, dim3(1), dim3(1024), 0, st, ctx->d_hist, ctx->d_off, ctx->d_choff, (uint32_t)nb_total, L0);
+      hipLaunchKernelGGL(k_scan_one, dim3(1), dim3(1024), 0, st, ctx->d_hist, ctx->d_off, ctx->d_choff, (uint32_t)nb_total, L0, ctx->d_zblock, zwords);
     } else {
       hipLaunchKernelGGL(k_scan1, dim3(nblk), dim3(256), 0, st, ctx->d_hist, ctx->d_off, ctx->d_choff, ctx->d_blocktot, (uint32_t)nb_total, L0);
-      hipLaunchKernelGGL(k_scan2, dim3(1), dim3(256), 0, st, ctx->d_blocktot, nblk, ctx->d_off, ctx->d_choff, (uint32_t)nb_total);
-      hipLaunchKernelGGL(k_scan3, dim3(nblk), dim3(256), 0, st, ctx->d_blocktot, ctx->d_off, ctx->d_choff, (uint32_t)nb_total);
+      hipLaunchKernelGGL(k_scan3, dim3(nblk), dim3(256), 0, st, ctx->d_blocktot, nblk, ctx->d_off, ctx->d_choff, (uint32_t)nb_total, ctx->d_zblock, zwords);
     }
   } else {
     HIPCHK(hipMemsetAsync(ctx->d_hist, 0, nb_total * 4, st));
     hipLaunchKernelGGL(k_hist, dim3(gn), dim3(256), 0, st, (const uint32_t*)d_scalars32, flags, ctx->d_hist, n32, plan, rank, world, bad_flag);
     if (profile >= 2) HIPCHK(hipEventRecord(ctx->ev[2], st));
     hipLaunchKernelGGL(k_scan1, dim3(nblk), dim3(256), 0, st, ctx->d_hist, ctx->d_off, ctx->d_choff, ctx->d_blocktot, (uint32_t)nb_total, L0);
-    hipLaunchKernelGGL(k_scan2, dim3(1), dim3(256), 0, st, ctx->d_blocktot, nblk, ctx->d_off, ctx->d_choff, (uint32_t)nb_total);
-    hipLaunchKernelGGL(k_scan3, dim3(nblk), dim3(256), 0, st, ctx->d_blocktot, ctx->d_off, ctx->d_choff, (uint32_t)nb_total);
+    hipLaunchKernelGGL(k_scan3, dim3(nblk), dim3(256), 0, st, ctx->d_blocktot, nblk, ctx->d_off, ctx->d_choff, (uint32_t)nb_total, ctx->d_zblock, zwords);
     if (profile >= 2) HIPCHK(hipEventRecord(ctx->ev[3], st));
     hipLaunchKernelGGL(k_scatter, dim3(gn), dim3(256), 0, st, (const uint32_t*)d_scalars32, flags, ctx->d_hist, ctx->d_off, ctx->d_sorted, n32, plan, rank, world);
   }
-  HIPCHK(hipMemsetAsync(ctx->d_zblock, 0, zblock_clear_bytes(ctx), st));
   hipLaunchKernelGGL(k_chunk_desc, dim3((uint32_t)std::min<size_t>(CHUNK_DESC_BLOCKS, (nb_total + 255) / 256)), dim3(256), 0, st, ctx->d_off, ctx->d_choff, ctx->d_desc, ctx->d_lenhist, ctx->d_heavy, (uint32_t)ctx->cap_heavy, (uint32_t)nb_total, L0, ctx->d_any_multi);
   const size_t max_chunks = nb_total + (n * (size_t)nlw) / L0 + 1;
   const uint32_t gchunks = (uint32_t)((max_chunks + 255) / 256);
-  hipLaunchKernelGGL(k_len_scan, dim3(1), dim3(256), 0, st, ctx->d_lenhist, ctx->d_lenhist + LEN_BINS, ctx->d_off + nb_total, ctx->d_choff + nb_total, bad_flag);
-  hipLaunchKernelGGL(k_order, dim3((gchunks + ORDER_PER - 1) / ORDER_PER), dim3(256), 0, st, ctx->d_desc, ctx->d_choff + nb_total, ctx->d_lenhist + LEN_BINS, ctx->d_order);
+  hipLaunchKernelGGL(k_order, dim3((gchunks + ORDER_PER - 1) / ORDER_PER), dim3(256), 0, st, ctx->d_desc, ctx->d_off + nb_total, ctx->d_choff + nb_total, ctx->d_lenhist,
+                     ctx->d_lenhist + LEN_BINS, ctx->d_order, bad_flag);
   if (hooks.before_accumulate) HIPCHK(hipStreamWaitEvent(st, hooks.before_accumulate, 0));
   if (profile >= 1) HIPCHK(hipEventRecord(ctx->ev[4], st));
   hipLaunchKernelGGL(k_accumulate, dim3(gchunks), dim3(256), 0, st, ctx->d_desc, ctx->d_choff + nb_total, ctx->d_order, ctx->d_sorted, pts, ctx->d_sums);
   if (profile >= 1) HIPCHK(hipEventRecord(ctx->ev[5], st));
   if (hooks.after_accumulate) HIPCHK(hipEventRecord(hooks.after_accumulate, st));
-  hipLaunchKernelGGL(k_heavy_combine, dim3(512), dim3(256), 0, st, ctx->d_heavy, (uint32_t)ctx->cap_heavy, ctx->d_choff, ctx->d_sums, ctx->d_combined);
   const bool small_quad = ctx->quad && ctx->rowcol_quad && nb_total <= (size_t)ctx->rowcol_quad_max;
   const bool rows_fold = small_quad && use2d && ctx->rowcol_row && ctx->tree_row && nb_total <= 8192;
-  if (rows_fold) {}
-  else if (small_quad && ctx->fold_quad)
+  const bool quad_fold = !rows_fold && small_quad && ctx->fold_quad;
+  const uint32_t nfold_blocks = (!rows_fold && !quad_fold && ctx->fold_pass) ? (uint32_t)((nb_total + 255) / 256) : 0u;
+  hipLaunchKernelGGL(k_chunk_join, dim3(HEAVY_BLOCKS + nfold_blocks), dim3(256), 0, st, ctx->d_heavy, (uint32_t)ctx->cap_heavy, ctx->d_choff, ctx->d_sums, ctx->d_combined,
+                     (uint32_t)nb_total, ctx->d_any_multi, HEAVY_BLOCKS);
+  if (quad_fold)
     hipLaunchKernelGGL(k_bucket_fold_quad, dim3((uint32_t)((nb_total * 4 + 255) / 256)), dim3(256), 0, st, ctx->d_choff, ctx->d_sums, ctx->d_combined, (uint32_t)nb_total, ctx->d_any_multi);
-  else if (ctx->fold_pass)
-    hipLaunchKernelGGL(k_bucket_fold, dim3((uint32_t)((nb_total + 255) / 256)), dim3(256), 0, st, ctx->d_choff, ctx->d_sums, ctx->d_combined, (uint32_t)nb_total, ctx->d_any_multi);
   bool tree_exports = false;
   if (use2d) {
     const uint32_t R = 1u << hb2, Cn = 1u << lb2;
@@ -659,23 +660,22 @@
   if (ctx->profile >= 2) HIPCHK(hipEventRecord(ctx->ev[2], st));
   const uint32_t nblk = (uint32_t)((nb_total + SCAN_ITEMS - 1) / SCAN_ITEMS);
   hipLaunchKernelGGL(k_scan1, dim3(nblk), dim3(256), 0, st, ctx->d_hist, ctx->d_off, ctx->d_choff, ctx->d_blocktot, (uint32_t)nb_total, L0);
-  hipLaunchKernelGGL(k_scan2, dim3(1), dim3(256), 0, st, ctx->d_blocktot, nblk, ctx->d_off, ctx->d_choff, (uint32_t)nb_total);
-  hipLaunchKernelGGL(k_scan3, dim3(nblk), dim3(256), 0, st, ctx->d_blocktot, ctx->d_off, ctx->d_choff, (uint32_t)nb_total);
+  hipLaunchKernelGGL(k_scan3, dim3(nblk), dim3(256), 0, st, ctx->d_blocktot, nblk, ctx->d_off, ctx->d_choff, (uint32_t)nb_total, ctx->d_zblock, zblock_clear_words(ctx));
   hipLaunchKernelGGL(k_group_scatter, dim3((uint32_t)M, nwin), dim3(256), 0, st, ctx->d_digits, ctx->d_boffs, ctx->d_off, ctx->d_sorted, Nv32, NB, nwin, split);
   if (ctx->profile >= 2) HIPCHK(hipEventRecord(ctx->ev[3], st));
-  HIPCHK(hipMemsetAsync(ctx->d_zblock, 0, zblock_clear_bytes(ctx), st));
   hipLaunchKernelGGL(k_chunk_desc, dim3((uint32_t)std::min<size_t>(CHUNK_DESC_BLOCKS, (nb_total + 255) / 256)), dim3(256), 0, st, ctx->d_off, ctx->d_choff, ctx->d_desc, ctx->d_lenhist, ctx->d_heavy, (uint32_t)ctx->cap_heavy, (uint32_t)nb_total, L0, ctx->d_any_multi);
   const size_t max_chunks = nb_total + (Nv * (size_t)nwin) / L0 + 1;
   const uint32_t gchunks = (uint32_t)((max_chunks + 255) / 256);
-  hipLaunchKernelGGL(k_len_scan, dim3(1), dim3(256), 0, st, ctx->d_lenhist, ctx->d_lenhist + LEN_BINS, ctx->d_off + nb_total, ctx->d_choff + nb_total, bad_flag);
-  hipLaunchKernelGGL(k_order, dim3((gchunks + ORDER_PER - 1) / ORDER_PER), dim3(256), 0, st, ctx->d_desc, ctx->d_choff + nb_total, ctx->d_lenhist + LEN_BINS, ctx->d_order);
+  hipLaunchKernelGGL(k_order, dim3((gchunks + ORDER_PER - 1) / ORDER_PER), dim3(256), 0, st, ctx->d_desc, ctx->d_off + nb_total, ctx->d_choff + nb_total, ctx->d_lenhist,
+                     ctx->d_lenhist + LEN_BINS, ctx->d_order, bad_flag);
   if (wait_before_accumulate) HIPCHK(hipStreamWaitEvent(st, wait_before_accumulate, 0));
   if (ctx->profile >= 1) HIPCHK(hipEventRecord(ctx->ev[4], st));
   hipLaunchKernelGGL(k_accumulate, dim3(gchunks), dim3(256), 0, st, ctx->d_desc, ctx->d_choff + nb_total, ctx->d_order, ctx->d_sorted, ctx->d_pts, ctx->d_sums);
   if (ctx->profile >= 1) HIPCHK(hipEventRecord(ctx->ev[5], st));
   if (record_after_accumulate) HIPCHK(hipEventRecord(record_after_accumulate, st));
   const uint32_t nseg_total = (uint32_t)(nb_total / m);
-  hipLaunchKernelGGL(k_heavy_combine, dim3(512), dim3(256), 0, st, ctx->d_heavy, (uint32_t)ctx->cap_heavy, ctx->d_choff, ctx->d_sums, ctx->d_combined);
+  hipLaunchKernelGGL(k_chunk_join, dim3(HEAVY_BLOCKS), dim3(256), 0, st, ctx->d_heavy, (uint32_t)ctx->cap_heavy, ctx->d_choff, ctx->d_sums, ctx->d_combined, (uint32_t)nb_total,
+                     ctx->d_any_multi, HEAVY_BLOCKS);
   hipLaunchKernelGGL(k_seg_reduce, dim3((nseg_total + 255) / 256), dim3(256), 0, st, ctx->d_choff, ctx->d_sums, ctx->d_combined, ctx->d_segrun, ctx->d_segtot, nseg_total, m);
   hipLaunchKernelGGL(k_group_reduce, dim3((uint32_t)((G + 255) / 256)), dim3(256), 0, st, ctx->d_segrun, ctx->d_segtot, ctx->d_gsum, (uint32_t)G, J, log2m);
   if (ctx->profile >= 2) HIPCHK(hipEventRecord(ctx->ev[6], st));
diff --git a/curdleproofs_pie_amd/csrc/host_context.h b/curdleproofs_pie_amd/csrc/host_context.h
--- a/curdleproofs_pie_amd/csrc/host_context.h
+++ b/curdleproofs_pie_amd/csrc/host_context.h
@@ -89,8 +89,8 @@
   PointSum* d_partial = nullptr; size_t cap_partial = 0;
   uint16_t* d_digits = nullptr; uint32_t* d_part = nullptr; uint32_t* d_blockcnt = nullptr; uint32_t* d_ublocktot = nullptr;
   size_t cap_digits = 0, cap_part = 0, cap_blockcnt = 0;
-  uint32_t *d_slice_base = nullptr, *d_slicehist = nullptr, *d_subbase = nullptr; uint8_t* d_bigflag = nullptr;
-  size_t cap_bigflag = 0, cap_slices = 0;
+  uint32_t *d_slice_base = nullptr, *d_slicehist = nullptr;
+  size_t cap_slice_bins = 0, cap_slices = 0;
   int big_bins = 1;
   int use_partition_sort = 1;
   int stage_sort = 1;
@@ -200,7 +200,7 @@
   c->d_lenhist = c->d_heavy = c->d_any_multi = nullptr; c->d_combined = nullptr; c->cap_zblock = 0; c->cap_heavy = 0; c->cap_combined = 0;
   c->cap_partial = 0;
   F(c->d_digits); F(c->d_part); F(c->d_blockcnt); F(c->d_ublocktot); F(c->d_boffs); F(c->d_gsum); F(c->d_bout);
-  F(c->d_slice_base); F(c->d_slicehist); F(c->d_subbase); F(c->d_bigflag); c->cap_bigflag = 0; c->cap_slices = 0;
+  F(c->d_slice_base); F(c->d_slicehist); c->cap_slice_bins = 0; c->cap_slices = 0;
   if (c->h_bout) { (void)hipHostFree(c->h_bout); c->h_bout = nullptr; }
   if (c->h_lin) { (void)hipHostFree(c->h_lin); c->h_lin = nullptr; c->h_lin_dev = nullptr; c->cap_h_lin = 0; }
   if (c->d_gout) { (void)hipFree(c->d_gout); c->d_gout = nullptr; }
@@ -249,7 +249,7 @@
   }
   {
     const size_t hcap = entries / ((size_t)L * (HEAVY_MIN_CHUNKS - 1)) + 2;
-    const size_t z0 = 2 * LEN_BINS + 1, h0 = z0 + (nb_total + 3) / 4, words = h0 + 1 + hcap + 64;
+    const size_t z0 = 2 * LEN_BINS + 1, h0 = z0 + (nb_total + 3) / 4, words = h0 + 1 + hcap;
     if (words > ctx->cap_zblock) {
       if (ctx->d_zblock) (void)hipFree(ctx->d_zblock);
       ctx->d_zblock = nullptr; ctx->cap_zblock = 0;
@@ -276,13 +276,11 @@
       HIPCHK(hipMalloc(&ctx->d_part, (entries + 1) * 4));
       ctx->cap_part = entries;
     }
-    if (nlw * 128 > ctx->cap_bigflag) {
+    if (nlw * 128 > ctx->cap_slice_bins) {
       auto F = [](auto*& p) { if (p) { (void)hipFree(p); p = nullptr; } };
-      F(ctx->d_bigflag); F(ctx->d_slice_base); F(ctx->d_subbase);
-      HIPCHK(hipMalloc(&ctx->d_bigflag, nlw * 128 + 16));
+      F(ctx->d_slice_base);
       HIPCHK(hipMalloc(&ctx->d_slice_base, (nlw * 128 + 1) * 4));
-      HIPCHK(hipMalloc(&ctx->d_subbase, nlw * 128 * 256 * 4));
-      ctx->cap_bigflag = nlw * 128;
+      ctx->cap_slice_bins = nlw * 128;
     }
     {
       const size_t max_slices = entries / SLICE + nlw * 128 + 1;
@@ -317,12 +315,7 @@
   return CG1_OK;
 }
 
-static size_t zblock_clear_bytes(const Ctx* ctx) {
-  size_t bytes = (size_t)((ctx->d_heavy + 1) - ctx->d_zblock) * 4;
-  bytes = (bytes + 255) & ~(size_t)255;
-  const size_t cap = ctx->cap_zblock * 4;
-  return bytes < cap ? bytes : cap;
-}
+static uint32_t zblock_clear_words(const Ctx* ctx) { return (uint32_t)((ctx->d_heavy + 1) - ctx->d_zblock); }
 
 static int read_phase_events(Ctx* ctx, int profile) {
   for (int i = 0; i < CG1_NPHASE; ++i) ctx->phase_ms[i] = 0.f;
diff --git a/curdleproofs_pie_amd/csrc/kernels_accumulate.h b/curdleproofs_pie_amd/csrc/kernels_accumulate.h
--- a/curdleproofs_pie_amd/csrc/kernels_accumulate.h
+++ b/curdleproofs_pie_amd/csrc/kernels_accumulate.h
@@ -48,13 +48,12 @@
   store_sum(sums + t, acc);
 }
 
-__global__ void __launch_bounds__(256) k_heavy_combine(const uint32_t* __restrict__ heavy, uint32_t heavy_cap,
-                                                       const uint32_t* __restrict__ choff, PointSum* __restrict__ sums,
-                                                       uint8_t* __restrict__ combined) {
+__device__ __forceinline__ void heavy_combine(const uint32_t* __restrict__ heavy, uint32_t heavy_cap, const uint32_t* __restrict__ choff,
+                                              PointSum* __restrict__ sums, uint8_t* __restrict__ combined, uint32_t nblocks) {
   __shared__ PointSum sh[4];
   uint32_t nheavy = heavy[0];
   if (nheavy > heavy_cap) nheavy = heavy_cap;
-  for (uint32_t h = blockIdx.x; h < nheavy; h += gridDim.x) {
+  for (uint32_t h = blockIdx.x; h < nheavy; h += nblocks) {
     const uint32_t b = heavy[1 + h];
     const uint32_t c0 = choff[b], c1 = choff[b + 1];
     xyzz acc = xyzz_identity();
@@ -75,10 +74,10 @@
   }
 }
 
-__global__ void __launch_bounds__(256) k_bucket_fold(const uint32_t* __restrict__ choff, PointSum* __restrict__ sums,
-                                                     uint8_t* __restrict__ combined, uint32_t nb_total, const uint32_t* __restrict__ any_multi = nullptr) {
+__device__ __forceinline__ void bucket_fold(const uint32_t* __restrict__ choff, PointSum* __restrict__ sums, uint8_t* __restrict__ combined,
+                                            uint32_t nb_total, const uint32_t* __restrict__ any_multi, uint32_t block) {
   if (any_multi && *any_multi == 0u) return;
-  uint32_t b = blockIdx.x * 256 + threadIdx.x;
+  uint32_t b = block * 256 + threadIdx.x;
   if (b >= nb_total) return;
   const uint32_t c0 = choff[b], c1 = choff[b + 1];
   if (c1 - c0 < 2u || c1 - c0 >= HEAVY_MIN_CHUNKS) return;
@@ -87,3 +86,11 @@
   store_sum(sums + c0, acc);
   combined[b] = 1;
 }
+
+constexpr uint32_t HEAVY_BLOCKS = 512;
+__global__ void __launch_bounds__(256) k_chunk_join(const uint32_t* __restrict__ heavy, uint32_t heavy_cap, const uint32_t* __restrict__ choff,
+                                                    PointSum* __restrict__ sums, uint8_t* __restrict__ combined, uint32_t nb_total,
+                                                    const uint32_t* __restrict__ any_multi, uint32_t nheavy_blocks) {
+  if (blockIdx.x < nheavy_blocks) heavy_combine(heavy, heavy_cap, choff, sums, combined, nheavy_blocks);
+  else bucket_fold(choff, sums, combined, nb_total, any_multi, blockIdx.x - nheavy_blocks);
+}
diff --git a/curdleproofs_pie_amd/csrc/kernels_sort.h b/curdleproofs_pie_amd/csrc/kernels_sort.h
--- a/curdleproofs_pie_amd/csrc/kernels_sort.h
+++ b/curdleproofs_pie_amd/csrc/kernels_sort.h
@@ -79,9 +79,74 @@
   if (threadIdx.x < nbins) block_counts[((size_t)lw * nbins + threadIdx.x) * nslices + slice] = cnt[threadIdx.x];
 }
 
+constexpr uint32_t PART_COUNT_THREADS = 1024;
+__global__ void __launch_bounds__(1024) k_part_count_scalars(const uint32_t* __restrict__ scalars, const uint8_t* __restrict__ inf_flag,
+                                                             uint16_t* __restrict__ digits, uint32_t* __restrict__ block_counts,
+                                                             uint32_t n, uint32_t nslices, uint32_t nbins, uint32_t sub_bits, uint32_t nlw,
+                                                             WinPlan pl, int rank, int world, uint32_t* __restrict__ bad_flag) {
+  extern __shared__ uint32_t pc_cnt[];
+  const uint32_t ncnt = nlw * nbins, slice = blockIdx.x;
+  for (uint32_t j = threadIdx.x; j < ncnt; j += PART_COUNT_THREADS) pc_cnt[j] = 0;
+  __syncthreads();
+  for (uint32_t k = 0; k < PART_TILE / PART_COUNT_THREADS; ++k) {
+    const uint32_t i = slice * PART_TILE + k * PART_COUNT_THREADS + threadIdx.x;
+    const bool in = i < n;
+    DigitIter it;
+    load_scalar(scalars, in ? i : 0u, it);
+    const bool skip = !in || inf_flag[i] != 0;
+    if (in && (it.s[7] >> 31)) *bad_flag = 1u;
+    WinWalk ww(rank, world);
+    for (int w = 0; w < pl.nwin; ++w) {
+      const int d = it.next(pl, w);
+      const int lw = ww.step(w);
+      if (lw < 0) continue;
+      const uint32_t e = skip ? 0u : (uint32_t)(d & 0xFFFF);
+      if (in) digits[(size_t)lw * n + i] = (uint16_t)e;
+      uint32_t neg;
+      const uint32_t key = e ? ((digit_mag(e, neg) - 1u) >> sub_bits) : 0u;
+      lds_ranked_inc(pc_cnt + (uint32_t)lw * nbins, key, e != 0u);
+    }
+  }
+  __syncthreads();
+  for (uint32_t j = threadIdx.x; j < ncnt; j += PART_COUNT_THREADS) block_counts[(size_t)j * nslices + slice] = pc_cnt[j];
+}
+
+constexpr uint32_t BIN_STAGE = 12288;
+constexpr uint32_t SLICE = BIN_STAGE;
+__device__ __forceinline__ void slice_plan(const uint32_t* __restrict__ block_base, uint32_t nbins_total, uint32_t nslices,
+                                           uint32_t* __restrict__ slice_base ) {
+  __shared__ uint32_t part_sum[256];
+  const uint32_t per = (nbins_total + 255u) / 256u, g0 = threadIdx.x * per;
+  uint32_t mine = 0;
+  for (uint32_t g = g0; g < g0 + per && g < nbins_total; ++g) {
+    const uint32_t size = block_base[(size_t)(g + 1) * nslices] - block_base[(size_t)g * nslices];
+    mine += size > BIN_STAGE ? (size + SLICE - 1u) / SLICE : 0u;
+  }
+  part_sum[threadIdx.x] = mine;
+  __syncthreads();
+  for (int d = 1; d < 256; d <<= 1) {
+    uint32_t u = ((int)threadIdx.x >= d) ? part_sum[threadIdx.x - d] : 0u;
+    __syncthreads();
+    part_sum[threadIdx.x] += u;
+    __syncthreads();
+  }
+  uint32_t run = part_sum[threadIdx.x] - mine;
+  for (uint32_t g = g0; g < g0 + per && g < nbins_total; ++g) {
+    const uint32_t size = block_base[(size_t)(g + 1) * nslices] - block_base[(size_t)g * nslices];
+    slice_base[g] = run;
+    run += size > BIN_STAGE ? (size + SLICE - 1u) / SLICE : 0u;
+  }
+  if (threadIdx.x == 255) slice_base[nbins_total] = part_sum[255];
+}
+
 __global__ void __launch_bounds__(256) k_part_scatter(const uint16_t* __restrict__ digits, const uint32_t* __restrict__ block_base,
                                                       uint32_t* __restrict__ part, uint32_t n, uint32_t nslices, uint32_t nbins,
-                                                      uint32_t sub_bits, int use_stage) {
+                                                      uint32_t sub_bits, int use_stage, uint32_t nbins_total,
+                                                      uint32_t* __restrict__ slice_base) {
+  if (blockIdx.y * nbins >= nbins_total) {
+    if (blockIdx.x == 0) slice_plan(block_base, nbins_total, nslices, slice_base);
+    return;
+  }
   __shared__ uint32_t cur[128];
   __shared__ uint32_t gbase[128];
   __shared__ uint32_t lbase[128];
@@ -130,85 +195,6 @@
     for (uint32_t o = threadIdx.x; o < total; o += 256) part[gpos[o]] = stage[o];
   }
 }
-constexpr uint32_t BIN_STAGE = 12288;
-__global__ void __launch_bounds__(256) k_bin_sort(const uint32_t* __restrict__ part, const uint32_t* __restrict__ block_base,
-                                                  uint32_t* __restrict__ hist, uint32_t* __restrict__ sorted,
-                                                  uint32_t nbins_total, uint32_t nslices, uint32_t sub_bits, int use_stage,
-                                                  const uint8_t* __restrict__ bigflag) {
-  __shared__ uint32_t cnt[256];
-  __shared__ uint32_t cur[256];
-  __shared__ uint32_t stage[BIN_STAGE];
-  const uint32_t g = blockIdx.x;
-  if (bigflag[g]) return;
-  const uint32_t start = block_base[(size_t)g * nslices];
-  const uint32_t end = block_base[(size_t)(g + 1) * nslices];
-  cnt[threadIdx.x] = 0;
-  __syncthreads();
-  const uint32_t span = ((end - start + 255u) / 256u) * 256u;
-  for (uint32_t o = threadIdx.x; o < span; o += 256) {
-    const bool live = start + o < end;
-    lds_ranked_inc(cnt, live ? (part[start + o] >> 24) : 0u, live);
-  }
-  __syncthreads();
-  const uint32_t mine = cnt[threadIdx.x];
-  cur[threadIdx.x] = mine;
-  __syncthreads();
-  for (int d = 1; d < 256; d <<= 1) {
-    uint32_t u = ((int)threadIdx.x >= d) ? cur[threadIdx.x - d] : 0u;
-    __syncthreads();
-    cur[threadIdx.x] += u;
-    __syncthreads();
-  }
-  const uint32_t excl = cur[threadIdx.x] - mine;
-  __syncthreads();
-  const bool staged = use_stage && (end - start) <= BIN_STAGE;
-  cur[threadIdx.x] = (staged ? 0u : start) + excl;
-  if (threadIdx.x < (1u << sub_bits)) hist[((size_t)g << sub_bits) + threadIdx.x] = mine;
-  __syncthreads();
-  for (uint32_t o = threadIdx.x; o < span; o += 256) {
-    const bool live = start + o < end;
-    const uint32_t v = live ? part[start + o] : 0u;
-    const uint32_t pos = lds_ranked_inc(cur, v >> 24, live);
-    const uint32_t val = (v & 0x7fffffu) | ((v >> 23 & 1u) << 31);
-    if (live) { if (staged) stage[pos] = val; else sorted[pos] = val; }
-  }
-  if (staged) {
-    __syncthreads();
-    for (uint32_t o = threadIdx.x; start + o < end; o += 256) sorted[start + o] = stage[o];
-  }
-}
-
-constexpr uint32_t SLICE = BIN_STAGE;
-
-__global__ void __launch_bounds__(256) k_slice_plan(const uint32_t* __restrict__ block_base, uint32_t nbins_total, uint32_t nslices,
-                                                    uint32_t* __restrict__ slice_base ,
-                                                    uint8_t* __restrict__ bigflag, int enable) {
-  __shared__ uint32_t part_sum[256];
-  const uint32_t per = (nbins_total + 255u) / 256u, g0 = threadIdx.x * per;
-  uint32_t mine = 0;
-  for (uint32_t g = g0; g < g0 + per && g < nbins_total; ++g) {
-    const uint32_t size = block_base[(size_t)(g + 1) * nslices] - block_base[(size_t)g * nslices];
-    mine += (enable && size > BIN_STAGE) ? (size + SLICE - 1u) / SLICE : 0u;
-  }
-  part_sum[threadIdx.x] = mine;
-  __syncthreads();
-  for (int d = 1; d < 256; d <<= 1) {
-    uint32_t u = ((int)threadIdx.x >= d) ? part_sum[threadIdx.x - d] : 0u;
-    __syncthreads();
-    part_sum[threadIdx.x] += u;
-    __syncthreads();
-  }
-  uint32_t run = part_sum[threadIdx.x] - mine;
-  for (uint32_t g = g0; g < g0 + per && g < nbins_total; ++g) {
-    const uint32_t size = block_base[(size_t)(g + 1) * nslices] - block_base[(size_t)g * nslices];
-    const uint32_t ns = (enable && size > BIN_STAGE) ? (size + SLICE - 1u) / SLICE : 0u;
-    slice_base[g] = run;
-    bigflag[g] = ns ? 1 : 0;
-    run += ns;
-  }
-  if (threadIdx.x == 255) slice_base[nbins_total] = part_sum[255];
-}
-
 __device__ __forceinline__ bool slice_of_block(const uint32_t* __restrict__ slice_base, uint32_t nbins_total, uint32_t b,
                                                uint32_t& g, uint32_t& s) {
   if (b >= slice_base[nbins_total]) return false;
@@ -222,12 +208,11 @@
   return true;
 }
 
-__global__ void __launch_bounds__(256) k_slice_count(const uint32_t* __restrict__ part, const uint32_t* __restrict__ block_base,
-                                                     uint32_t nbins_total, uint32_t nslices, const uint32_t* __restrict__ slice_base,
-                                                     uint32_t* __restrict__ slicehist) {
-  __shared__ uint32_t cnt[256];
+__device__ __forceinline__ void slice_count(const uint32_t* __restrict__ part, const uint32_t* __restrict__ block_base,
+                                            uint32_t nbins_total, uint32_t nslices, const uint32_t* __restrict__ slice_base,
+                                            uint32_t* __restrict__ slicehist, uint32_t b, uint32_t* cnt) {
   uint32_t g, s;
-  if (!slice_of_block(slice_base, nbins_total, blockIdx.x, g, s)) return;
+  if (!slice_of_block(slice_base, nbins_total, b, g, s)) return;
   const uint32_t start = block_base[(size_t)g * nslices], end = block_base[(size_t)(g + 1) * nslices];
   const uint32_t lo = start + s * SLICE, hi = (lo + SLICE < end) ? lo + SLICE : end;
   cnt[threadIdx.x] = 0;
@@ -238,40 +223,61 @@
     lds_ranked_inc(cnt, live ? (part[lo + o] >> 24) : 0u, live);
   }
   __syncthreads();
-  slicehist[(size_t)blockIdx.x * 256u + threadIdx.x] = cnt[threadIdx.x];
-}
-
-__global__ void __launch_bounds__(256) k_slice_prefix(const uint32_t* __restrict__ block_base, uint32_t nslices, uint32_t sub_bits,
-                                                      const uint32_t* __restrict__ slice_base, const uint8_t* __restrict__ bigflag,
-                                                      uint32_t* __restrict__ slicehist, uint32_t* __restrict__ subbase,
-                                                      uint32_t* __restrict__ hist) {
-  __shared__ uint32_t tot[256];
+  slicehist[(size_t)b * 256u + threadIdx.x] = cnt[threadIdx.x];
+}
+
+__global__ void __launch_bounds__(256) k_bin_sort(const uint32_t* __restrict__ part, const uint32_t* __restrict__ block_base,
+                                                  uint32_t* __restrict__ hist, uint32_t* __restrict__ sorted,
+                                                  uint32_t nbins_total, uint32_t nslices, uint32_t sub_bits, int use_stage,
+                                                  int big_bins, const uint32_t* __restrict__ slice_base, uint32_t* __restrict__ slicehist) {
+  __shared__ uint32_t cnt[256];
+  __shared__ uint32_t cur[256];
+  __shared__ uint32_t stage[BIN_STAGE];
   const uint32_t g = blockIdx.x;
-  if (!bigflag[g]) return;
-  const uint32_t b0 = slice_base[g], b1 = slice_base[g + 1];
-  uint32_t run = 0;
-  for (uint32_t b = b0; b < b1; ++b) {
-    const size_t idx = (size_t)b * 256u + threadIdx.x;
-    const uint32_t v = slicehist[idx];
-    slicehist[idx] = run;
-    run += v;
-  }
-  tot[threadIdx.x] = run;
+  if (g >= nbins_total) { slice_count(part, block_base, nbins_total, nslices, slice_base, slicehist, g - nbins_total, cnt); return; }
+  const uint32_t start = block_base[(size_t)g * nslices];
+  const uint32_t end = block_base[(size_t)(g + 1) * nslices];
+  if (big_bins && end - start > BIN_STAGE) return;
+  cnt[threadIdx.x] = 0;
+  __syncthreads();
+  const uint32_t span = ((end - start + 255u) / 256u) * 256u;
+  for (uint32_t o = threadIdx.x; o < span; o += 256) {
+    const bool live = start + o < end;
+    lds_ranked_inc(cnt, live ? (part[start + o] >> 24) : 0u, live);
+  }
+  __syncthreads();
+  const uint32_t mine = cnt[threadIdx.x];
+  cur[threadIdx.x] = mine;
   __syncthreads();
   for (int d = 1; d < 256; d <<= 1) {
-    uint32_t u = ((int)threadIdx.x >= d) ? tot[threadIdx.x - d] : 0u;
-    __syncthreads();
-    tot[threadIdx.x] += u;
-    __syncthreads();
-  }
-  subbase[(size_t)g * 256u + threadIdx.x] = block_base[(size_t)g * nslices] + tot[threadIdx.x] - run;
-  if (threadIdx.x < (1u << sub_bits)) hist[((size_t)g << sub_bits) + threadIdx.x] = run;
+    uint32_t u = ((int)threadIdx.x >= d) ? cur[threadIdx.x - d] : 0u;
+    __syncthreads();
+    cur[threadIdx.x] += u;
+    __syncthreads();
+  }
+  const uint32_t excl = cur[threadIdx.x] - mine;
+  __syncthreads();
+  const bool staged = use_stage && (end - start) <= BIN_STAGE;
+  cur[threadIdx.x] = (staged ? 0u : start) + excl;
+  if (threadIdx.x < (1u << sub_bits)) hist[((size_t)g << sub_bits) + threadIdx.x] = mine;
+  __syncthreads();
+  for (uint32_t o = threadIdx.x; o < span; o += 256) {
+    const bool live = start + o < end;
+    const uint32_t v = live ? part[start + o] : 0u;
+    const uint32_t pos = lds_ranked_inc(cur, v >> 24, live);
+    const uint32_t val = (v & 0x7fffffu) | ((v >> 23 & 1u) << 31);
+    if (live) { if (staged) stage[pos] = val; else sorted[pos] = val; }
+  }
+  if (staged) {
+    __syncthreads();
+    for (uint32_t o = threadIdx.x; start + o < end; o += 256) sorted[start + o] = stage[o];
+  }
 }
 
 __global__ void __launch_bounds__(256) k_slice_scatter(const uint32_t* __restrict__ part, const uint32_t* __restrict__ block_base,
-                                                       uint32_t nbins_total, uint32_t nslices, const uint32_t* __restrict__ slice_base,
-                                                       const uint32_t* __restrict__ slicehist, const uint32_t* __restrict__ subbase,
-                                                       uint32_t* __restrict__ sorted) {
+                                                       uint32_t nbins_total, uint32_t nslices, uint32_t sub_bits,
+                                                       const uint32_t* __restrict__ slice_base, const uint32_t* __restrict__ slicehist,
+                                                       uint32_t* __restrict__ hist, uint32_t* __restrict__ sorted) {
   __shared__ uint32_t cnt[256];
   __shared__ uint32_t cur[256];
   __shared__ uint32_t gdst[256];
@@ -298,9 +304,25 @@
   }
   const uint32_t lbase = cnt[threadIdx.x] - mine;
   __syncthreads();
+  uint32_t before = 0, tot = 0;
+  for (uint32_t b = blockIdx.x - s, b1 = slice_base[g + 1]; b < b1; ++b) {
+    const uint32_t v = slicehist[(size_t)b * 256u + threadIdx.x];
+    before += b < blockIdx.x ? v : 0u;
+    tot += v;
+  }
+  cur[threadIdx.x] = tot;
+  __syncthreads();
+  for (int d = 1; d < 256; d <<= 1) {
+    uint32_t u = ((int)threadIdx.x >= d) ? cur[threadIdx.x - d] : 0u;
+    __syncthreads();
+    cur[threadIdx.x] += u;
+    __syncthreads();
+  }
+  gdst[threadIdx.x] = start + cur[threadIdx.x] - tot + before;
+  if (s == 0 && threadIdx.x < (1u << sub_bits)) hist[((size_t)g << sub_bits) + threadIdx.x] = tot;
+  __syncthreads();
   cnt[threadIdx.x] = lbase;
   cur[threadIdx.x] = lbase;
-  gdst[threadIdx.x] = subbase[(size_t)g * 256u + threadIdx.x] + slicehist[(size_t)blockIdx.x * 256u + threadIdx.x];
   __syncthreads();
   for (uint32_t o = threadIdx.x; o < span; o += 256) {
     const bool live = lo + o < hi;
@@ -315,6 +337,15 @@
   }
 }
 
+__device__ __forceinline__ uint32_t block_sum256(uint32_t v, uint32_t* sh) {
+  for (int d = 32; d >= 1; d >>= 1) v += __shfl_xor(v, d, 64);
+  if ((threadIdx.x & 63u) == 0u) sh[threadIdx.x >> 6] = v;
+  __syncthreads();
+  v = sh[0] + sh[1] + sh[2] + sh[3];
+  __syncthreads();
+  return v;
+}
+
 __global__ void __launch_bounds__(256) k_uscan1(uint32_t* __restrict__ a, uint32_t* __restrict__ block_tot, uint32_t n) {
   __shared__ uint32_t sh[256];
   uint32_t base = blockIdx.x * SCAN_ITEMS + threadIdx.x * 4;
@@ -334,32 +365,20 @@
   for (int k = 0; k < 4; ++k) { if (base + k < n) a[base + k] = excl; excl += v[k]; }
   if (threadIdx.x == 255) block_tot[blockIdx.x] = sh[255];
 }
-__global__ void __launch_bounds__(256) k_uscan2(uint32_t* __restrict__ block_tot, uint32_t nblocks, uint32_t* __restrict__ a, uint32_t n) {
-  __shared__ uint32_t sh[256];
-  uint32_t carry = 0;
-  for (uint32_t tile = 0; tile < nblocks; tile += 256) {
-    uint32_t i = tile + threadIdx.x;
-    uint32_t v = (i < nblocks) ? block_tot[i] : 0u;
-    sh[threadIdx.x] = v;
-    __syncthreads();
-    for (int d = 1; d < 256; d <<= 1) {
-      uint32_t u = ((int)threadIdx.x >= d) ? sh[threadIdx.x - d] : 0u;
-      __syncthreads();
-      sh[threadIdx.x] += u;
-      __syncthreads();
-    }
-    if (i < nblocks) block_tot[i] = carry + sh[threadIdx.x] - v;
-    uint32_t tot = sh[255];
-    __syncthreads();
-    carry += tot;
-  }
-  if (threadIdx.x == 0) a[n] = carry;
-}
-__global__ void __launch_bounds__(256) k_uscan3(const uint32_t* __restrict__ block_tot, uint32_t* __restrict__ a, uint32_t n) {
+__global__ void __launch_bounds__(256) k_uscan3(const uint32_t* __restrict__ block_tot, uint32_t nblocks, uint32_t* __restrict__ a, uint32_t n) {
+  __shared__ uint32_t sh[4];
+  uint32_t p = 0;
+  for (uint32_t i = threadIdx.x; i < blockIdx.x; i += 256) p += block_tot[i];
+  p = block_sum256(p, sh);
   uint32_t base = blockIdx.x * SCAN_ITEMS + threadIdx.x * 4;
-  uint32_t p = block_tot[blockIdx.x];
 #pragma unroll
   for (int k = 0; k < 4; ++k) if (base + k < n) a[base + k] += p;
+  if (blockIdx.x == gridDim.x - 1) {
+    uint32_t t = 0;
+    for (uint32_t i = blockIdx.x + threadIdx.x; i < nblocks; i += 256) t += block_tot[i];
+    t = block_sum256(t, sh);
+    if (threadIdx.x == 0) a[n] = p + t;
+  }
 }
 
 constexpr uint32_t USCAN1_MAX = 1u << 15;
@@ -493,35 +512,23 @@
   }
   if (threadIdx.x == 255) block_tot[blockIdx.x] = sh[255];
 }
-__global__ void __launch_bounds__(256) k_scan2(uint2* __restrict__ block_tot, uint32_t nblocks, uint32_t* __restrict__ off,
-                                               uint32_t* __restrict__ choff, uint32_t nb_total) {
-  __shared__ uint2 sh[256];
-  uint2 carry = make_uint2(0, 0);
-  for (uint32_t tile = 0; tile < nblocks; tile += 256) {
-    uint32_t i = tile + threadIdx.x;
-    uint2 v = (i < nblocks) ? block_tot[i] : make_uint2(0, 0);
-    sh[threadIdx.x] = v;
-    __syncthreads();
-    for (int d = 1; d < 256; d <<= 1) {
-      uint2 u = make_uint2(0, 0);
-      if ((int)threadIdx.x >= d) u = sh[threadIdx.x - d];
-      __syncthreads();
-      sh[threadIdx.x].x += u.x; sh[threadIdx.x].y += u.y;
-      __syncthreads();
-    }
-    if (i < nblocks) block_tot[i] = make_uint2(carry.x + sh[threadIdx.x].x - v.x, carry.y + sh[threadIdx.x].y - v.y);
-    uint2 tot = sh[255];
-    __syncthreads();
-    carry.x += tot.x; carry.y += tot.y;
-  }
-  if (threadIdx.x == 0) { off[nb_total] = carry.x; choff[nb_total] = carry.y; }
-}
-__global__ void __launch_bounds__(256) k_scan3(const uint2* __restrict__ block_tot, uint32_t* __restrict__ off,
-                                               uint32_t* __restrict__ choff, uint32_t nb_total) {
+__global__ void __launch_bounds__(256) k_scan3(const uint2* __restrict__ block_tot, uint32_t nblocks, uint32_t* __restrict__ off,
+                                               uint32_t* __restrict__ choff, uint32_t nb_total,
+                                               uint32_t* __restrict__ zero, uint32_t zero_words) {
+  __shared__ uint32_t sh[4];
+  for (uint32_t i = blockIdx.x * 256 + threadIdx.x; i < zero_words; i += gridDim.x * 256) zero[i] = 0;
+  uint2 p = make_uint2(0, 0);
+  for (uint32_t i = threadIdx.x; i < blockIdx.x; i += 256) { const uint2 v = block_tot[i]; p.x += v.x; p.y += v.y; }
+  p.x = block_sum256(p.x, sh); p.y = block_sum256(p.y, sh);
   uint32_t base = blockIdx.x * SCAN_ITEMS + threadIdx.x * 4;
-  uint2 p = block_tot[blockIdx.x];
 #pragma unroll
   for (int k = 0; k < 4; ++k) if (base + k < nb_total) { off[base + k] += p.x; choff[base + k] += p.y; }
+  if (blockIdx.x == gridDim.x - 1) {
+    uint2 t = make_uint2(0, 0);
+    for (uint32_t i = blockIdx.x + threadIdx.x; i < nblocks; i += 256) { const uint2 v = block_tot[i]; t.x += v.x; t.y += v.y; }
+    t.x = block_sum256(t.x, sh); t.y = block_sum256(t.y, sh);
+    if (threadIdx.x == 0) { off[nb_total] = p.x + t.x; choff[nb_total] = p.y + t.y; }
+  }
 }
 
 constexpr uint32_t LEN_BINS = 256;
@@ -529,8 +536,9 @@
 
 constexpr uint32_t SCAN1_MAX = 1u << 13;
 __global__ void __launch_bounds__(1024) k_scan_one(const uint32_t* __restrict__ hist, uint32_t* __restrict__ off, uint32_t* __restrict__ choff,
-                                                    uint32_t nb_total, uint32_t L0) {
+                                                    uint32_t nb_total, uint32_t L0, uint32_t* __restrict__ zero, uint32_t zero_words) {
   __shared__ uint2 sh[1024];
+  for (uint32_t i = threadIdx.x; i < zero_words; i += 1024) zero[i] = 0;
   const uint32_t per = (nb_total + 1023u) / 1024u, lo = threadIdx.x * per, hi = (lo + per < nb_total) ? lo + per : nb_total;
   uint2 local = make_uint2(0, 0);
   for (uint32_t i = lo; i < hi; ++i) { const uint32_t c = hist[i]; local.x += c; local.y += chunk_count(c, L0); }
@@ -586,14 +594,20 @@
   if (v) atomicAdd(&len_hist[threadIdx.x], v);
 }
 
-__global__ void __launch_bounds__(256) k_len_scan(const uint32_t* __restrict__ len_hist, uint32_t* __restrict__ len_cursor,
-                                                  const uint32_t* __restrict__ total_entries, const uint32_t* __restrict__ total_chunks,
-                                                  uint32_t* __restrict__ stats) {
+constexpr uint32_t ORDER_PER = 8;
+__global__ void __launch_bounds__(256) k_order(const uint2* __restrict__ desc, const uint32_t* __restrict__ total_entries,
+                                               const uint32_t* __restrict__ total_chunks, const uint32_t* __restrict__ len_hist,
+                                               uint32_t* __restrict__ len_cursor, uint32_t* __restrict__ order, uint32_t* __restrict__ stats) {
+  __shared__ uint32_t cnt[LEN_BINS];
+  __shared__ uint32_t base[LEN_BINS];
   __shared__ uint32_t sh[LEN_BINS];
-  if (threadIdx.x == 0) { stats[1] = *total_entries; stats[2] = *total_chunks; }
-  uint32_t rev = LEN_BINS - 1 - threadIdx.x;
-  uint32_t v = len_hist[rev];
-  sh[threadIdx.x] = v;
+  const uint32_t total = *total_chunks;
+  if (blockIdx.x == 0 && threadIdx.x == 0) { stats[1] = *total_entries; stats[2] = total; }
+  if (blockIdx.x * ORDER_PER * 256u >= total) return;
+  cnt[threadIdx.x] = 0;
+  const uint32_t rev = LEN_BINS - 1 - threadIdx.x;
+  const uint32_t hv = len_hist[rev];
+  sh[threadIdx.x] = hv;
   __syncthreads();
   for (int d = 1; d < 256; d <<= 1) {
     uint32_t u = ((int)threadIdx.x >= d) ? sh[threadIdx.x - d] : 0u;
@@ -601,17 +615,7 @@
     sh[threadIdx.x] += u;
     __syncthreads();
   }
-  len_cursor[rev] = sh[threadIdx.x] - v;
-}
-
-constexpr uint32_t ORDER_PER = 8;
-__global__ void __launch_bounds__(256) k_order(const uint2* __restrict__ desc, const uint32_t* __restrict__ total_chunks,
-                                               uint32_t* __restrict__ len_cursor, uint32_t* __restrict__ order) {
-  __shared__ uint32_t cnt[LEN_BINS];
-  __shared__ uint32_t base[LEN_BINS];
-  cnt[threadIdx.x] = 0;
-  __syncthreads();
-  const uint32_t total = *total_chunks;
+  base[rev] = sh[threadIdx.x] - hv;
   uint32_t key[ORDER_PER], local[ORDER_PER];
 #pragma unroll
   for (uint32_t rep = 0; rep < ORDER_PER; ++rep) {
@@ -633,7 +637,7 @@
   }
   __syncthreads();
   const uint32_t c = cnt[threadIdx.x];
-  if (c) base[threadIdx.x] = atomicAdd(&len_cursor[threadIdx.x], c);
+  if (c) base[threadIdx.x] += atomicAdd(&len_cursor[threadIdx.x], c);
   __syncthreads();
 #pragma unroll
   for (uint32_t rep = 0; rep < ORDER_PER; ++rep) {
```

Result: no change. 370.8 million (-0.2%).
